# infergo-ml/gogp

Hardware: AMD Instinct MI355X
Metric: GP.Observe+Gradient evals/sec (fp64) at N=16384 D=8 (higher is better)
Workload: dtype f64

## Files before the change

gogp_amd/_lib.py:

```python
from __future__ import annotations

import ctypes
import os
import subprocess

from .kernel import CDesc

_HERE = os.path.dirname(os.path.abspath(__file__))
LIB_PATH = os.path.join(_HERE, "libgogp_hip.so")
HOOKS_PATH = os.path.join(_HERE, "libgogp_testhooks.so")

GOGP_OK, GOGP_EARG, GOGP_ENOTPD, GOGP_EHIP, GOGP_ESTATE, GOGP_ENOMEM, GOGP_ECOND = 0, 1, 2, 3, 4, 5, 6
GOGP_MAX_CANDIDATES = 16
GOGP_BATCH_MAX_N = 128
GOGP_COV_MAX_M = 4096

_dp = ctypes.POINTER(ctypes.c_double)
_i64 = ctypes.c_int64
_h = ctypes.c_void_p
_descp = ctypes.POINTER(CDesc)
GOGP_UNIQUE_ID_BYTES = 128


class CXfer(ctypes.Structure):
    _fields_ = [("peer", ctypes.c_int32), ("is_send", ctypes.c_int32), ("buf", ctypes.c_void_p),
                ("bytes", ctypes.c_int64)]


EXCHANGE_FN = ctypes.CFUNCTYPE(ctypes.c_int, ctypes.c_void_p, ctypes.POINTER(CXfer), ctypes.c_int32)
ALLREDUCE_FN = ctypes.CFUNCTYPE(ctypes.c_int, ctypes.c_void_p, ctypes.POINTER(ctypes.c_double),
                                ctypes.c_int64)
class CGemmOpts(ctypes.Structure):
    _fields_ = [(n, ctypes.c_int32) for n in ("ktri", "krag0", "new_row0", "kbeg0", "small_below", "prio", "rule",
                                              "tpb_shift", "rblk0", "cblk0", "pr", "Pr", "pc", "Pc", "beta0", "k")]
    _fields_ += [("bstride", ctypes.c_int64)]
    DEFAULTS = dict(ktri=0, krag0=-1, new_row0=-1, kbeg0=0, small_below=384, prio=0, rule=0, tpb_shift=0, rblk0=0,
                    cblk0=0, pr=0, Pr=1, pc=0, Pc=1, beta0=-1, k=1, bstride=0)


class CKParams(ctypes.Structure):
    _T, _D, _E = 4, 64, 32
    _fields_ = [("ndim", ctypes.c_int32), ("nterms", ctypes.c_int32), ("kind", ctypes.c_int32 * _T),
                ("ard", ctypes.c_int32 * _T), ("c", ctypes.c_double * _T), ("w", ctypes.c_double * _T),
                ("inv_len", (ctypes.c_double * _D) * _T), ("noise_var", ctypes.c_double), ("dnoise", ctypes.c_double),
                ("nevents", ctypes.c_int32), ("ev_axis", ctypes.c_int32), ("ev_from", ctypes.c_double * _E),
                ("ev_to", ctypes.c_double * _E), ("ev_disc", ctypes.c_double * _E)]


GOGP_TEST_NACC = 16 + 64


class CGemmPlan(ctypes.Structure):
    _fields_ = [("tile", ctypes.c_int32), ("waves", ctypes.c_int32), ("grid_x", ctypes.c_int64),
                ("grid_z", ctypes.c_int64), ("flops", ctypes.c_double), ("tag", ctypes.c_int64)]


SYMBOLS = [
    ("gogp_desc_check", ctypes.c_int, [_descp]),
    ("gogp_desc_ntheta_noise", ctypes.c_int, [_descp]),
    ("gogp_create", ctypes.c_int, [_descp, ctypes.c_int, ctypes.POINTER(_h)]),
    ("gogp_destroy", None, [_h]),
    ("gogp_last_error", ctypes.c_char_p, [_h]),
    ("gogp_notpd_index", _i64, [_h]),
    ("gogp_graph_info", ctypes.c_int, [_h, ctypes.POINTER(ctypes.c_int64), ctypes.POINTER(ctypes.c_int)]),
    ("gogp_events_check", ctypes.c_int, [_dp, ctypes.c_int, ctypes.c_int, ctypes.c_int]),
    ("gogp_set_events", ctypes.c_int, [_h, _dp, ctypes.c_int, ctypes.c_int]),
    ("gogp_set_data", ctypes.c_int, [_h, _dp, _dp, _i64]),
    ("gogp_set_data_device", ctypes.c_int, [_h, ctypes.c_void_p, ctypes.c_void_p, _i64]),
    ("gogp_absorb", ctypes.c_int, [_h, _dp, _dp]),
    ("gogp_observe", ctypes.c_int, [_h, _dp, _i64, _dp]),
    ("gogp_observe_full", ctypes.c_int, [_h, _dp, _i64, _dp]),
    ("gogp_lml", ctypes.c_int, [_h, _dp]),
    ("gogp_gradient", ctypes.c_int, [_h, _dp, _i64]),
    ("gogp_loo", ctypes.c_int, [_h, _dp, _dp, _dp, _dp]),
    ("gogp_loo_gradient", ctypes.c_int, [_h, _dp, _i64]),
    ("gogp_observe_gradient_batch", ctypes.c_int,
     [ctypes.POINTER(_h), ctypes.c_int, _dp, _i64, _dp, _dp, ctypes.POINTER(ctypes.c_int)]),
    ("gogp_observe_gradient_candidates", ctypes.c_int,
     [_h, ctypes.c_int, _dp, _i64, _dp, _dp, ctypes.POINTER(ctypes.c_int)]),
    ("gogp_batch_set_data", ctypes.c_int,
     [_h, _dp, _dp, _i64, ctypes.c_int32, ctypes.POINTER(_i64), ctypes.POINTER(_i64)]),
    ("gogp_batch_observe_gradient", ctypes.c_int,
     [_h, ctypes.c_int32, ctypes.POINTER(ctypes.c_int32), _dp, _i64, _dp, _dp, ctypes.POINTER(ctypes.c_int)]),
    ("gogp_batch_produce", ctypes.c_int,
     [_h, ctypes.c_int32, ctypes.POINTER(ctypes.c_int32), _dp, _i64, ctypes.POINTER(_i64), _dp, _dp, _dp, _dp,
      ctypes.POINTER(ctypes.c_int)]),
    ("gogp_batch_observe_full_gradient", ctypes.c_int,
     [_h, ctypes.c_int32, _dp, ctypes.POINTER(_i64), _dp, _dp, ctypes.POINTER(ctypes.c_int)]),
    ("gogp_batch_produce_full", ctypes.c_int,
     [_h, ctypes.c_int32, _dp, ctypes.POINTER(_i64), ctypes.POINTER(_i64), _dp, _dp, _dp, _dp,
      ctypes.POINTER(ctypes.c_int)]),
    ("gogp_produce", ctypes.c_int, [_h, _dp, _i64, _dp, _dp]),
    ("gogp_produce_gradient", ctypes.c_int, [_h, _dp, _i64, _dp, _dp, _dp, _dp]),
    ("gogp_produce_covariance", ctypes.c_int, [_h, _dp, _i64, _dp, _dp]),
    ("gogp_produce_samples", ctypes.c_int, [_h, _dp, _i64, _dp, _i64, ctypes.c_double, _dp, _dp]),
    ("gogp_n", _i64, [_h]),
    ("gogp_get_alpha", ctypes.c_int, [_h, _dp]),
    ("gogp_get_factor", ctypes.c_int, [_h, _dp]),
    ("gogp_get_factor_rows", ctypes.c_int, [_h, ctypes.POINTER(_i64), _i64, _dp]),
    ("gogp_get_factor_diag", ctypes.c_int, [_h, _dp]),
    ("gogp_set_factor", ctypes.c_int, [_h, _dp, _dp, _dp, _dp]),
    ("gogp_append", ctypes.c_int, [_h, _dp, _dp, ctypes.c_int64]),
    ("gogp_remove", ctypes.c_int, [_h, ctypes.POINTER(_i64), ctypes.c_int64]),
    ("gogp_dist_grid", ctypes.c_int, [ctypes.c_int, ctypes.POINTER(ctypes.c_int), ctypes.POINTER(ctypes.c_int)]),
    ("gogp_dist_unique_id", ctypes.c_int, [ctypes.c_void_p]),
    ("gogp_dist_init_rccl", ctypes.c_int,
     [_h, ctypes.c_int, ctypes.c_int, ctypes.c_int, ctypes.c_int, ctypes.c_char_p]),
    ("gogp_dist_init_callbacks", ctypes.c_int,
     [_h, ctypes.c_int, ctypes.c_int, ctypes.c_int, ctypes.c_int, ctypes.c_void_p, ctypes.c_void_p,
      ctypes.c_void_p]),
    ("gogp_dist_local_bytes", _i64, [_h]),
    ("gogp_dist_comm_ranks", ctypes.c_int, [_h, ctypes.POINTER(ctypes.c_int)]),
    ("gogp_dist_selftest", ctypes.c_int, [_h, ctypes.c_int, _i64]),
    ("gogp_profile_enable", ctypes.c_int, [_h, ctypes.c_int]),
    ("gogp_profile_read", ctypes.c_int, [_h, _dp, ctypes.POINTER(_i64), _dp, _dp]),
    ("gogp_profile_read_launches", ctypes.c_int,
     [_h, _i64, _dp, _dp, _dp, ctypes.POINTER(_i64), ctypes.POINTER(_i64)]),
    ("gogp_profile_read_aux", ctypes.c_int, [_h, ctypes.c_int, _dp, ctypes.POINTER(_i64)]),
    ("gogp_set_option", ctypes.c_int, [_h, ctypes.c_char_p, _i64]),
    ("gogp_version", ctypes.c_char_p, []),
]

HOOK_SYMBOLS = [
    ("gogp_mfma_f64_peak", ctypes.c_int, [ctypes.c_int, ctypes.c_int, _dp, _dp, _dp]),
    ("gogp_mfma_f32_peak", ctypes.c_int, [ctypes.c_int, ctypes.c_int, _dp, _dp, _dp]),
    ("gogp_bench_gemm", ctypes.c_int,
     [ctypes.c_int, ctypes.c_int, ctypes.c_int, ctypes.c_int, _i64, ctypes.c_int, _dp, _dp]),
    ("gogp_test_diag256", ctypes.c_int,
     [ctypes.c_int, _dp, _dp, _dp, ctypes.POINTER(ctypes.c_uint64), _dp]),
    ("gogp_test_dgemm_nt", ctypes.c_int,
     [ctypes.c_int, _i64, _i64, _i64, ctypes.c_double, _dp, _dp, ctypes.c_double, _dp]),
    ("gogp_test_valu_cost", ctypes.c_int, [ctypes.c_int, _dp]),
    ("gogp_test_panel128", ctypes.c_int,
     [ctypes.c_int, _dp, _dp, _i64, ctypes.c_int, ctypes.POINTER(ctypes.c_uint64), _dp]),
    ("gogp_test_panel128_slabs", ctypes.c_int, [ctypes.c_int, _dp, _dp, _i64, ctypes.c_int, ctypes.c_int, _dp]),
    ("gogp_test_gemm_nt", ctypes.c_int,
     [ctypes.c_int, ctypes.c_int, ctypes.c_int, ctypes.c_int, ctypes.c_int, _i64, ctypes.c_double, ctypes.c_double]
# ... 90 lines not shown
```

gogp_amd/csrc/api.hip:

```cpp
#include <math.h>
#include <stdio.h>
#include <stdlib.h>
#include <string.h>

#include <algorithm>
#include <initializer_list>
#include <mutex>
#include <new>
#include <thread>
#include <type_traits>
#include <utility>

#include "handle.h"

using namespace gogp;

static thread_local std::string g_create_error;

extern "C" int gogp_desc_ntheta_noise(const gogp_desc *d) {
  return (d && (d->noise_kind == GOGP_NOISE_UNIFORM || d->noise_kind == GOGP_NOISE_CONSTANT_PARAM)) ? 1 : 0;
}

extern "C" int gogp_desc_check(const gogp_desc *d) {
  if (!d) return GOGP_EARG;
// ... 537 lines not shown
  int P0, nsub, prevP0, next_nsub;
  int64_t C0() const { return (int64_t)P0 * PANEL; }
  int64_t CE() const { return C0() + (int64_t)nsub * PANEL; }
};
static std::vector<SuperPanel> superpanels(const gogp_handle *h) {
  const int npanel = (int)(h->npad / PANEL);
  std::vector<SuperPanel> v;
  for (int P0 = 0; P0 < npanel; P0 += v.back().nsub) {
    const int nsub = superpanel_width(h, npanel, P0);
    if (!v.empty()) v.back().next_nsub = nsub;
    v.push_back({P0, nsub, v.empty() ? -1 : v.back().P0, 0});
  }
  return v;
}
struct InnerGroup {
  int grp;
  int64_t k0, ce;
};
static inline InnerGroup inner_group(int q, int64_t c2, int64_t CE) {
  const int done = q + 1, grp = done & -done;
  return {grp, c2 - (int64_t)grp * PANEL, std::min(c2 + (int64_t)grp * PANEL, CE)};
}

constexpr int TMT_BLOCKS = 8;
static inline int tinv_panels(const gogp_handle *h) { return h->produce_panels; }
static inline int64_t tinv_signature(const gogp_handle *h) {
  return (int64_t)h->produce_panels + (h->npad << 8) + ((int64_t)h->prec << 56);
}
static int ensure_tinv(gogp_handle *h) {
  const int64_t tld = (int64_t)tinv_panels(h) * PANEL;
  const size_t need = (size_t)std::max(h->npad, h->cap_npad) * (size_t)tld;
  if (!h->TX || h->cap_tinv < need) {
    (void)hipFree(h->TX);
    (void)hipFree(h->Tmt);
    h->TX = h->Tmt = nullptr;
    h->cap_tinv = 0;
    HIPCHK(h, hipMalloc(&h->TX, need * h->esz()));
    HIPCHK(h, hipMalloc(&h->Tmt, (size_t)TMT_BLOCKS * PANEL * PANEL * h->esz()));
    h->cap_tinv = need;
  }
  h->tinv_ld = tld;
  return GOGP_OK;
}

template <class T>
static void assemble_tinv(gogp_handle *h, hipStream_t sp, int P0, int nsub) {
  const int64_t ld = h->npad, tld = h->tinv_ld, C0 = (int64_t)P0 * PANEL;
  T *X = reinterpret_cast<T *>(h->TX) + C0 * tld;
  T *MT = reinterpret_cast<T *>(h->Tmt);
  const T *L = reinterpret_cast<const T *>(h->bufL);
  const T *Dinv = reinterpret_cast<const T *>(h->Dinv) + (size_t)P0 * PANEL * PANEL;
  launch_tinv_init(sp, Dinv, X, (T *)nullptr, nsub, tld);
  for (int d = 1; d < nsub; ++d) {
    const int cnt = nsub - d;
    for (int b0 = 0; b0 < cnt; b0 += 6) {
      const int nb = std::min(6, cnt - b0);
      const T *A1[6], *B1[6], *A2[6], *B2[6];
      T *C1[6], *C2[6];
      int64_t lda1[6], ldb1[6], ldc1[6], lda2[6], ldb2[6], ldc2[6];
      int K1[6], K2[6];
      for (int b = 0; b < nb; ++b) {
        const int i = d + b0 + b, j = i - d;
        A1[b] = L + (C0 + (int64_t)i * PANEL) * ld + C0 + (int64_t)j * PANEL;
        lda1[b] = ld;
        B1[b] = X + (int64_t)j * PANEL * tld + (int64_t)j * PANEL;
        ldb1[b] = tld;
        C1[b] = MT + (size_t)(b0 + b) * PANEL * PANEL;
        ldc1[b] = PANEL;
        K1[b] = d * PANEL;
        A2[b] = Dinv + (size_t)i * PANEL * PANEL;
        lda2[b] = PANEL;
        B2[b] = C1[b];
        ldb2[b] = PANEL;
        C2[b] = X + (int64_t)i * PANEL * tld + (int64_t)j * PANEL;
        ldc2[b] = tld;
        K2[b] = PANEL;
      }
      launch_blockmm(sp, nb, A1, lda1, B1, ldb1, C1, ldc1, K1, 1.0);
      launch_blockmm(sp, nb, A2, lda2, B2, ldb2, C2, ldc2, K2, -1.0);
    }
  }
}

template <class T>
struct InvBufs {
  T *A, *Y;
  const T *L, *Dinv;
};
template <class T>
static void trtri_superstep(gogp_handle *h, const InvBufs<T> &B, const SuperPanel &P, hipStream_t st, hipStream_t s2) {
  const int64_t npad = h->npad, ld = npad;
  T *R = B.A, *Y = B.Y;
  const T *L = B.L;
  GemmProfile *pf = &h->prof;
  const int P0 = P.P0;
  const int64_t C0 = P.C0(), CE = P.CE();
  for (int q = 0; q < P.nsub; ++q) {
    const int p = P0 + q;
    const int64_t c0 = (int64_t)p * PANEL, c2 = c0 + PANEL;
    const T *Dp = B.Dinv + (size_t)p * PANEL * PANEL;
    launch_ydiag(st, Dp, Y + c0 * ld + c0, ld);
    if (c2 < CE)
      launch_zero_block(st, Y + c2 * ld + c0, ld, CE - c2, PANEL);
    if (c0 > 0) {
      GemmGrid gtri = chain_grid(h);
      gtri.ktri = h->ktri;
      launch_gemm_nt(st, GEMM_RECT, (int)(c0 / TILE), 2, PANEL, 1.0, R + c0, ld, Dp, PANEL, 0.0,
                      Y + c0, ld, pf, &gtri);
    }
    if (c2 < CE) {
      const InnerGroup g = inner_group(q, c2, CE);
      GemmGrid gch = chain_grid(h);
      if (h->krag) gch.krag0 = (int)(g.k0 / TILE);
      launch_gemm_nt(st, GEMM_RECT, (int)(c2 / TILE), (int)((g.ce - c2) / TILE), (int64_t)g.grp * PANEL,
                      -1.0, Y + g.k0, ld, L + c2 * ld + g.k0, ld, 1.0, R + c2, ld, pf, &gch);
    }
  }
  order(h, EV_BASE + 4 * P0 + 2, st, s2);
  const int nt = (int)((npad - CE) / TILE);
  if (nt > 0) {
    const int64_t Kw = CE - C0;
    const int mr = (int)(CE / TILE);
    const int ntn = nt < 2 * P.next_nsub ? nt : 2 * P.next_nsub;
    if (P0 > 0 && st != s2)
      (void)gogp::rec_stream_wait(st, ev(h, EV_BASE + 4 * P.prevP0 + 3));
    GemmGrid gch = chain_grid(h), gbulk;
    if (h->krag) gch.krag0 = gbulk.krag0 = (int)(C0 / TILE);
    launch_gemm_nt(st, GEMM_RECT, mr, ntn, Kw, -1.0, Y + C0, ld, L + CE * ld + C0, ld, 1.0,
                    R + CE, ld, pf, &gch);
    if (nt > ntn) {
      const int64_t C3 = CE + (int64_t)ntn * TILE;
      launch_gemm_nt(s2, GEMM_RECT, mr, nt - ntn, Kw, -1.0, Y + C0, ld, L + C3 * ld + C0, ld, 1.0,
                      R + C3, ld, pf, &gbulk);
    }
    (void)gogp::rec_event_record(ev(h, EV_BASE + 4 * P0 + 3), s2);
  }
}

static inline bool mixed_gradient(const gogp_handle *h) {
  return h->grad_prec == 32 && h->prec == 64 && !h->batch_mode && !h->dist;
}
static int ensure_g32(gogp_handle *h) {
  const int64_t cap = std::max(h->npad, h->cap_npad);
  if (h->g32A && h->g32_cap >= cap) return GOGP_OK;
  (void)hipFree(h->g32A);
  (void)hipFree(h->g32L);
  (void)hipFree(h->g32Y);
  (void)hipFree(h->g32D);
  h->g32A = h->g32L = h->g32Y = h->g32D = nullptr;
  h->g32_cap = 0;
  const size_t nn = (size_t)cap * (size_t)cap * sizeof(float);
  HIPCHK(h, hipMalloc(&h->g32A, nn));
  HIPCHK(h, hipMalloc(&h->g32L, nn));
  HIPCHK(h, hipMalloc(&h->g32Y, nn));
  HIPCHK(h, hipMalloc(&h->g32D, (size_t)(cap / PANEL) * PANEL * PANEL * sizeof(float)));
  h->g32_cap = cap;
  return GOGP_OK;
}
static void mixed_superstep(gogp_handle *h, const SuperPanel &P, hipStream_t st, hipStream_t s2) {
  const int64_t npad = h->npad, ld = npad, C0 = P.C0(), W = P.CE() - C0;
  launch_convert_block(st, h->bufL + C0 * ld + C0, ld, h->g32L + C0 * ld + C0, ld, (int)(npad - C0), (int)W);
  launch_convert_block(st, h->Dinv + (size_t)P.P0 * PANEL * PANEL, PANEL, h->g32D + (size_t)P.P0 * PANEL * PANEL, PANEL,
                       (int)W, PANEL);
  const InvBufs<float> B{h->g32A, h->g32Y, h->g32L, h->g32D};
  trtri_superstep<float>(h, B, P, st, s2);
}

template <class T>
static void kinv_accumulate(gogp_handle *h, const T *Y, T *A, int64_t C0, int64_t CE) {
  (void)gogp::rec_stream_wait(h->sk, ev(h, EV_BASE + 4 * (size_t)(C0 / PANEL) + 2));
  GemmGrid gk;
  gk.new_row0 = (int)(C0 / TILE);
  if (h->krag) gk.krag0 = (int)(C0 / TILE);
  launch_gemm_nt(h->sk, GEMM_LOWER, (int)(CE / TILE), (int)(CE / TILE), CE - C0, 1.0, Y + C0, h->npad, Y + C0, h->npad,
                 1.0, A, h->npad, &h->prof, &gk);
}

template <class T>
static void zero_inverse_rhs(gogp_handle *h, bool mixed, hipStream_t s) {
  if (mixed)
    launch_zero_upper_blocks(s, h->g32A, h->npad, h->npad);
  else
    launch_zero_upper_blocks(s, reinterpret_cast<T *>(h->bufA), h->npad, h->npad);
}
template <class T>
static void inverse_superstep(gogp_handle *h, bool mixed, const SuperPanel &P, hipStream_t st, hipStream_t s2,
                              bool fuse_kinv) {
  if (mixed) {
    mixed_superstep(h, P, st, s2);
    if (fuse_kinv) kinv_accumulate<float>(h, h->g32Y, h->g32A, P.C0(), P.CE());
  } else {
    const InvBufs<T> B{reinterpret_cast<T *>(h->bufA), reinterpret_cast<T *>(h->bufY), reinterpret_cast<const T *>(h->bufL),
                       reinterpret_cast<const T *>(h->Dinv)};
    trtri_superstep<T>(h, B, P, st, s2);
    if (fuse_kinv) kinv_accumulate<T>(h, B.Y, B.A, P.C0(), P.CE());
  }
}

static inline int chain_split_of(const gogp_handle *h, bool eager) {
  if (h->dist || h->prec != 64) return 0;
  if (h->chain_split >= 0) return h->chain_split;
  return (h->npad <= 8192 || !eager) ? 2 : 0;
}
static void fused_panel(gogp_handle *h, hipStream_t sp, double *A, double *L, int64_t ld, int64_t c0, int64_t npad,
                        GemmProfile *pf) {
  const int64_t c1 = c0 + TILE, c2 = c0 + PANEL;
  const int mt1 = (int)((npad - c1) / TILE);
  const GemmGrid gch = chain_grid(h);
  launch_panel128_slabs(sp, A + c0 * ld + c0, ld, L + c0 * ld + c0, ld, 0, npad - c1, c0, h->n, h->info, h->chain_slabs);
  launch_gemm_nt(sp, GEMM_RECT, mt1, 1, TILE, -1.0, L + c1 * ld + c0, ld, L + c1 * ld + c0, ld, 1.0, A + c1 * ld + c1, ld,
                 pf, &gch);
  launch_panel128_slabs(sp, A + c0 * ld + c0, ld, L + c0 * ld + c0, ld, 1, npad - c2, c0, h->n, h->info, h->chain_slabs);
}

static void begin_evaluation(gogp_handle *h, std::initializer_list<hipStream_t> streams) {
  auto wait = [&](int e) {
    for (hipStream_t q : streams) (void)gogp::rec_stream_wait(q, ev(h, e));
  };
  if (h->trtri_pending) wait(EV_TRTRI);
  if (h->kinv_pending) wait(EV_KINV);
  if (h->kinv_c1 > 0 && !h->have_kinv) wait(EV_KINV);
  h->trtri_pending = h->kinv_pending = false;
  h->factored = h->have_alpha = h->have_kinv = h->grad_valid = false;
  h->alpha_pending = h->trtri_done = h->ydone_valid = h->d64_active = false;
  h->notpd = -1;
  h->kinv_c1 = 0;
  if (!h->batch_mode) h->tinv_valid = false;
}
static hipError_t enqueue_result_scalars(gogp_handle *h, hipStream_t s) {
  const hipError_t e = cand_d2h(h, h->hscal, h->scalars, 7 * sizeof(double), s);
  return e != hipSuccess ? e : cand_d2h(h, h->hscal + HS_INFO, h->info, sizeof(long long), s);
}

template <class T>
static void substitute_fwd(gogp_handle *h, hipStream_t q, const T *L, const T *Dinv, double *w, double *dst) {
  const int npanel = (int)(h->npad / PANEL);
  for (int b = 0; b < npanel; ++b) launch_trsv_fwd_step(q, L, h->npad, Dinv, b, npanel, w, dst);
}
template <class T>
static hipError_t substitute_bwd(gogp_handle *h, hipStream_t q, const T *L, const T *Dinv, const double *src, double *w,
                                 double *dst) {
  const int npanel = (int)(h->npad / PANEL);
  const hipError_t e = hipMemcpyAsync(w, src, (size_t)h->npad * sizeof(double), hipMemcpyDeviceToDevice, q);
  for (int b = npanel - 1; b >= 0 && e == hipSuccess; --b) launch_trsv_bwd_step(q, L, h->npad, Dinv, b, npanel, w, dst);
  return e;
}

template <class T>
struct Sweep {
  static constexpr bool fp32 = sizeof(T) == 4;
  gogp_handle *h;
  bool eager;
  T *A = reinterpret_cast<T *>(h->bufA), *L = reinterpret_cast<T *>(h->bufL), *Dinv = reinterpret_cast<T *>(h->Dinv);
  int64_t npad = h->npad, ld = npad;
  int npanel = (int)(npad / PANEL);
  GemmProfile *pf = &h->prof;
  hipStream_t s = h->s, st = h->st, s2 = h->s2;
  hipStream_t sp = h->lookahead ? h->sp : h->s;
  hipStream_t sz = h->lookahead ? h->sl : sp;
  bool mixed = !fp32 && mixed_gradient(h);
  bool fuse_kinv = eager && (h->kinv_fused < 0 ? (npad <= 10240 || mixed) : h->kinv_fused != 0);
  int split = fp32 ? 0 : chain_split_of(h, eager);

  void d64_init(hipStream_t q, int first, int nblk) const {
    if constexpr (fp32)
      launch_widen_diag_blocks(q, A + (int64_t)first * PANEL * (ld + 1), ld, h->D64 + (size_t)first * PANEL * PANEL, nblk);
  }
  void d64_update(hipStream_t q, int64_t k0, int64_t K, int first, int nblk) const {
    if constexpr (fp32) {
      if (h->d64_active)
        launch_diag_syrk_f64(q, L + (int64_t)first * PANEL * ld + k0, ld, K, h->D64 + (size_t)first * PANEL * PANEL, nblk);
    }
  }

  int build_gram() const {
    if (sp != s) order(h, EV_ENTRY, s, sp);
    HIPCHK(h, cand_memset(h, h->info, sizeof(long long), sp));
    const int w0 = superpanel_width(h, npanel, 0);
    {
      AuxTimer tm(h, GOGP_PROF_GRAM, s);
      launch_gram_lower_split(sp, s, h->devP, h->D, h->dX, h->n, npad, A, ld, (int64_t)w0 * PANEL, h->ev());
    }
    h->d64_active = fp32 && h->diag_fp64 != 0;
    if (h->d64_active) {
      const int rc = ensure_d64(h);
      if (rc != GOGP_OK) return rc;
      d64_init(sp, 0, w0);
      if (npanel > w0) d64_init(s, w0, npanel - w0);
    }
    (void)gogp::rec_event_record(ev(h, EV_GRAM), s);
    if (eager) {
      (void)gogp::rec_stream_wait(s2, ev(h, EV_GRAM));
      (void)gogp::rec_stream_wait(st, ev(h, EV_GRAM));
      zero_inverse_rhs<T>(h, mixed, s2);
      order(h, EV_INIT, s2, st);
    }
    return GOGP_OK;
  }

  void chain_superpanel(const SuperPanel &P) const {
    const int64_t CE = P.CE();
    for (int q = 0; q < P.nsub; ++q) {
      const int p = P.P0 + q;
      const int64_t c0 = (int64_t)p * PANEL, c2 = c0 + PANEL;
      if constexpr (!fp32) {
        if (split) fused_panel(h, sp, A, L, ld, c0, npad, pf);
      }
      if (!split) {
        T *Dp = Dinv + (size_t)p * PANEL * PANEL;
        diag_block(h, sp, A + c0 * ld + c0, ld, L + c0 * ld + c0, ld, Dp, c0);
        const int mt2 = (int)((npad - c2) / TILE);
        if (mt2 > 0) {
          GemmGrid gtri = chain_grid(h);
          gtri.ktri = h->ktri;
          launch_gemm_nt(sp, GEMM_RECT, mt2, 2, PANEL, 1.0, A + c2 * ld + c0, ld, Dp, PANEL, 0.0,
                          L + c2 * ld + c0, ld, pf, &gtri);
        }
      }
      if (c2 < CE) {
        d64_update(sp, c0, PANEL, p + 1, (int)((CE - c2) / PANEL));
        const InnerGroup g = inner_group(q, c2, CE);
        const GemmGrid gch = chain_grid(h);
        launch_gemm_nt(sp, GEMM_TRAP, (int)((npad - c2) / TILE), (int)((g.ce - c2) / TILE),
                        (int64_t)g.grp * PANEL, -1.0, L + c2 * ld + g.k0, ld, L + c2 * ld + g.k0, ld, 1.0,
                        A + c2 * ld + c2, ld, pf, &gch);
      }
    }
  }

  void panels_final(const SuperPanel &P) const {
    order(h, EV_BASE + 4 * P.P0, sp, s);
    if (sz != sp) (void)gogp::rec_stream_wait(sz, ev(h, EV_BASE + 4 * P.P0));
    if constexpr (!fp32) {
      if (split) {
        launch_dinv256_blocks(sz, L + (int64_t)P.P0 * PANEL * (ld + 1), ld, Dinv + (size_t)P.P0 * PANEL * PANEL, P.nsub);
        if (eager) {
          (void)gogp::rec_event_record(ev(h, EV_BASE + 5 * (size_t)npanel + 32 + (size_t)P.P0), sz);
          (void)gogp::rec_stream_wait(st, ev(h, EV_BASE + 5 * (size_t)npanel + 32 + (size_t)P.P0));
        }
      }
    }
    for (int q = 0; q < P.nsub; ++q) launch_trsv_fwd_step(sz, L, ld, Dinv, P.P0 + q, npanel, h->w, h->z);
  }

  void trailing_update(const SuperPanel &P) const {
    const int64_t C0 = P.C0(), CE = P.CE();
    const int mtE = (int)((npad - CE) / TILE);
    if (mtE <= 0) return;
    const int64_t Kw = CE - C0;
    const int ntn = mtE < 2 * P.next_nsub ? mtE : 2 * P.next_nsub;
    (void)gogp::rec_stream_wait(sp, ev(h, P.P0 > 0 ? EV_BASE + 4 * P.prevP0 + 1 : EV_GRAM));
    const GemmGrid gch = chain_grid(h);
    launch_gemm_nt(sp, GEMM_TRAP, mtE, ntn, Kw, -1.0, L + CE * ld + C0, ld, L + CE * ld + C0, ld,
                    1.0, A + CE * ld + CE, ld, pf, &gch);
    d64_update(sp, C0, Kw, (int)(CE / PANEL), ntn / 2);
    if (mtE > ntn) {
      const int64_t C3 = CE + (int64_t)ntn * TILE;
      launch_gemm_nt(s, GEMM_LOWER, mtE - ntn, mtE - ntn, Kw, -1.0, L + C3 * ld + C0, ld,
                      L + C3 * ld + C0, ld, 1.0, A + C3 * ld + C3, ld, pf);
      d64_update(s, C0, Kw, (int)(C3 / PANEL), (mtE - ntn) / 2);
    }
    (void)gogp::rec_event_record(ev(h, EV_BASE + 4 * P.P0 + 1), s);
  }

  void inverse_behind(const SuperPanel &P) const {
    const int64_t CE = P.CE();
    (void)gogp::rec_stream_wait(st, ev(h, EV_BASE + 4 * P.P0));
    inverse_superstep<T>(h, mixed, P, st, s2, fuse_kinv);
    if (!fp32 && !fuse_kinv && !mixed && !h->batch_mode && h->kinv_split > 0 && h->kinv_c1 == 0 && CE < npad &&
        CE * 100 >= npad * (int64_t)h->kinv_split) {
      (void)gogp::rec_stream_wait(h->sk, ev(h, EV_BASE + 4 * P.P0 + 2));
      const T *Y0 = reinterpret_cast<const T *>(h->bufY);
      launch_gemm_nt(h->sk, GEMM_LAUUM, (int)(CE / TILE), (int)(CE / TILE), CE, 1.0, Y0, ld, Y0, ld, 0.0, A, ld, pf);
      (void)gogp::rec_event_record(ev(h, EV_KINV), h->sk);
      h->kinv_c1 = CE;
    }
  }

  int finish_alpha() const {
    if (fp32) {
      if (sz != sp) (void)gogp::rec_stream_wait(sp, ev(h, EV_FWD));
      HIPCHK(h, substitute_bwd(h, sp, L, Dinv, h->z, h->w, h->alpha));
      for (int it = 0; it < h->refine_steps; ++it) {
        launch_residual(sp, h->devP, h->D, h->dX, h->n, npad, h->alpha, h->dy, h->rpart, REFINE_SLABS, h->rw,
                        h->radial1, h->ev());
        substitute_fwd(h, sp, L, Dinv, h->rw, h->rz);
        HIPCHK(h, substitute_bwd(h, sp, L, Dinv, h->rz, h->rw, h->rd));
        launch_axpy(sp, h->alpha, h->rd, npad);
      }
      launch_dot(sp, h->dy, h->alpha, h->n, h->scalars + 6);
      order(h, EV_ALPHA, sp, s);
    }
    HIPCHK(h, enqueue_result_scalars(h, s));
    if (fp32) {
      if (eager) (void)gogp::rec_event_record(ev(h, EV_TRTRI), st);
    } else if (eager && !mixed) {
      (void)gogp::rec_stream_wait(st, ev(h, EV_FWD));
      launch_alpha_from_y(st, reinterpret_cast<const T *>(h->bufY), ld, h->z, npad, h->alpha);
      (void)gogp::rec_event_record(ev(h, EV_ALPHA), st);
      (void)gogp::rec_event_record(ev(h, EV_TRTRI), st);
    } else {
      if (sz != sp) (void)gogp::rec_stream_wait(sp, ev(h, EV_FWD));
      HIPCHK(h, substitute_bwd(h, sp, L, Dinv, h->z, h->w, h->alpha));
      (void)gogp::rec_event_record(ev(h, EV_ALPHA), sp);
    }
    return GOGP_OK;
  }
};

template <class T>
static int factorize_t(gogp_handle *h, bool eager) {
  const Sweep<T> c{h, eager && h->lookahead != 0};
  begin_evaluation(h, {c.s, c.sp});
  int rc = gogp_upload_params(h);
  if (rc == GOGP_OK && (c.mixed || c.eager)) rc = c.mixed ? ensure_g32(h) : ensure_y(h);
  if (rc == GOGP_OK) rc = c.build_gram();
  if (rc != GOGP_OK) return rc;
  if (c.fp32) HIPCHK(h, hipMemsetAsync(h->scalars + 5, 0, sizeof(double), c.sp));
  HIPCHK(h, cand_copy_in(h, h->w, h->dy, (size_t)c.npad * sizeof(double), c.sp));
  if (c.sz != c.sp) order(h, EV_W, c.sp, c.sz);
  for (const SuperPanel &P : superpanels(h)) {
    c.chain_superpanel(P);
    c.panels_final(P);
    c.trailing_update(P);
    if (c.eager) c.inverse_behind(P);
  }
  if (c.fuse_kinv) {
    (void)gogp::rec_event_record(ev(h, EV_KINV), h->sk);
    h->kinv_pending = true;
  }
  if (c.eager) {
    (void)gogp::rec_event_record(ev(h, EV_TRTRI), c.st);
    (void)gogp::rec_event_record(ev(h, EV_YDONE), c.st);
    h->ydone_valid = h->trtri_done = h->trtri_pending = true;
  }
  order(h, EV_FWD, c.sz, c.s);
  launch_lml_scalars(c.s, c.L, c.ld, h->z, nullptr, nullptr, h->n, h->scalars);
  rc = c.finish_alpha();
  if (rc != GOGP_OK) return rc;
  const int rcf = finish_factorize(h, c.fp32, c.fp32, false);
  if (rcf == GOGP_ENOTPD)
    for (hipStream_t q : {c.sp, c.st, c.s2, h->sl, h->sk}) (void)hipStreamSynchronize(q);
  return rcf;
}

static inline bool tiny_ok(const gogp_handle *h) {
  return h->tiny && !h->dist && h->prec == 64 && h->npad == PANEL && h->n <= TILE && !mixed_gradient(h);
}
static int tiny_factorize(gogp_handle *h, bool eager) {
  hipStream_t s = h->s;
  begin_evaluation(h, {s});
  int rc = gogp_upload_params(h);
  if (rc != GOGP_OK) return rc;
  if (h->lookahead && !h->batch_mode) {
    order(h, EV_ENTRY, h->sp, s);
    order(h, EV_W, h->sl, s);
  }
  HIPCHK(h, cand_memset(h, h->info, sizeof(long long), s));
  launch_tiny_eval(s, h->devP, h->dX, h->dy, h->n, h->bufA, h->bufL, h->Dinv, h->z, h->alpha, h->info, eager, h->ev());
  launch_lml_scalars(s, h->bufL, h->npad, h->z, nullptr, nullptr, h->n, h->scalars);
  (void)gogp::rec_event_record(ev(h, EV_ALPHA), s);
  HIPCHK(h, enqueue_result_scalars(h, s));
  return finish_factorize(h, false, false, eager);
}

static int factorize(gogp_handle *h, bool eager) {
  if (tiny_ok(h)) return tiny_factorize(h, eager && h->lookahead);
  return h->prec == 32 ? factorize_t<float>(h, eager) : factorize_t<double>(h, eager);
}

static int ensure_alpha(gogp_handle *h) {
  if (!h->factored || !h->have_alpha) return fail(h, GOGP_ESTATE, "no factorisation");
  if (h->alpha_pending) {
    HIPCHK(h, gogp::rec_stream_wait(h->s, ev(h, EV_ALPHA)));
    h->alpha_pending = false;
  }
  return GOGP_OK;
}

static const char *theta_refusal(const gogp_handle *h, const double *ts, const double *tn) {
  for (int i = 0; i < h->ns; ++i)
    if (!(ts[i] > 0.0) || !std::isfinite(ts[i])) return "similarity parameters must be positive and finite";
  for (int i = 0; i < h->nn; ++i)
    if (!std::isfinite(tn[i])) return "noise parameter must be finite";
  return nullptr;
}

static int set_theta_natural(gogp_handle *h, const double *ts, const double *tn) {
  if (const char *why = theta_refusal(h, ts, tn)) return fail(h, GOGP_EARG, why);
  for (int i = 0; i < h->ns; ++i) h->theta_s[i] = ts[i];
  for (int i = 0; i < h->nn; ++i) h->theta_n[i] = tn[i];
  h->have_theta = true;
  return GOGP_OK;
}

extern "C" int gogp_absorb(gogp_handle *h, const double *theta_simil,
                           const double *theta_noise) {
  if (!h || !theta_simil || (h->nn > 0 && !theta_noise)) return fail(h, GOGP_EARG, "absorb: NULL");
  if (!h->have_data) return fail(h, GOGP_ESTATE, "absorb: no data (gogp_set_data)");
  HIPCHK(h, hipSetDevice(h->device));
  int rc = set_theta_natural(h, theta_simil, theta_noise);
// ... 7 lines not shown
    return GOGP_OK;
  }
  rc = h->dist ? gogp_dist_factorize(h, false) : factorize(h, false);
  if (rc != GOGP_OK && rc != GOGP_ECOND) return rc;
  const int rcond = rc;
  rc = ensure_alpha(h);
  if (rc != GOGP_OK) return rc;
  HIPCHK(h, hipStreamSynchronize(h->s));
  return rcond;
}

static int observe_theta(gogp_handle *h, const double *x, double *lml) {
  std::vector<double> th(h->P > 0 ? h->P : 1);
  for (int i = 0; i < h->P; ++i) th[i] = exp(x[i]);
  int rc = set_theta_natural(h, th.data(), th.data() + h->ns);
  if (rc != GOGP_OK) return rc;
  h->grad_valid = false;
  if (h->n == 0) {
    h->lml = 0.0;
    h->factored = false;
    h->observed = true;
    if (lml) *lml = 0.0;
    return GOGP_OK;
  }
  rc = h->dist ? gogp_dist_factorize(h, true)
               : factorize(h, h->eager != 0);
  if (rc != GOGP_OK && rc != GOGP_ECOND) return rc;
  h->observed = true;
  if (lml) *lml = h->lml;
  return rc;
}

extern "C" int gogp_observe(gogp_handle *h, const double *x, int64_t len, double *lml) {
  if (!h || !x) return fail(h, GOGP_EARG, "observe: NULL");
  if (len != h->P) return fail(h, GOGP_EARG, "len(x)");
  if (!h->have_data) return fail(h, GOGP_ESTATE, "observe: no data (gogp_set_data)");
  HIPCHK(h, hipSetDevice(h->device));
  h->with_obs = false;
  return observe_theta(h, x, lml);
}

extern "C" int gogp_observe_full(gogp_handle *h, const double *x, int64_t len, double *lml) {
  if (!h || !x) return fail(h, GOGP_EARG, "observe: NULL");
  if (len < h->P) return fail(h, GOGP_EARG, "len(x)");
  const int64_t rest = len - h->P;
  if (rest == 0) return gogp_observe(h, x, len, lml);
  const int64_t n = rest / (h->D + 1);
  if (n * (h->D + 1) != rest) return fail(h, GOGP_EARG, "len(x)");
  int rc = gogp_set_data(h, x + h->P, x + h->P + n * h->D, n);
  if (rc != GOGP_OK) return rc;
  h->with_obs = true;
  return observe_theta(h, x, lml);
}

extern "C" int gogp_lml(gogp_handle *h, double *lml) {
  if (!h || !lml) return GOGP_EARG;
  if (h->n == 0) {
    *lml = 0.0;
    return GOGP_OK;
  }
  if (!h->factored) return fail(h, GOGP_ESTATE, "LML: nothing absorbed");
  *lml = h->lml;
  return GOGP_OK;
}

template <class T>
static int compute_kinv_t(gogp_handle *h) {
  if (h->have_kinv) return GOGP_OK;
  const int64_t npad = h->npad, ld = npad;
  hipStream_t s = h->s;
  GemmProfile *pf = &h->prof;
  if (h->kinv_pending) {
    (void)gogp::rec_stream_wait(s, ev(h, EV_KINV));
    if (h->trtri_pending) (void)gogp::rec_stream_wait(s, ev(h, EV_TRTRI));
    h->kinv_pending = h->trtri_pending = false;
    h->have_kinv = true;
    return GOGP_OK;
  }
  const bool mixed = std::is_same<T, double>::value && mixed_gradient(h);
  if (!h->trtri_done) {
    hipStream_t sp = h->lookahead ? h->sp : h->s;
    const int rcy = mixed ? ensure_g32(h) : ensure_y(h);
    if (rcy != GOGP_OK) return rcy;
    zero_inverse_rhs<T>(h, mixed, s);
    order(h, EV_INIT, s, sp);
    for (const SuperPanel &P : superpanels(h)) inverse_superstep<T>(h, mixed, P, sp, s, false);
    order(h, EV_TRTRI, sp, s);
    h->trtri_done = true;
  } else if (h->trtri_pending) {
    (void)gogp::rec_stream_wait(s, ev(h, h->ydone_valid ? EV_YDONE : EV_TRTRI));
  }
  if (mixed) {
    launch_gemm_nt(s, GEMM_LAUUM, h->nblk, h->nblk, npad, 1.0, h->g32Y, ld, h->g32Y, ld, 0.0, h->g32A, ld, pf);
  } else {
    GemmGrid gk;
    if (h->kinv_c1 > 0) {
      (void)gogp::rec_stream_wait(s, ev(h, EV_KINV));
      gk.kbeg0 = (int)h->kinv_c1;
    }
    launch_gemm_nt(s, GEMM_LAUUM, h->nblk, h->nblk, npad, 1.0, reinterpret_cast<const T *>(h->bufY), ld,
                   reinterpret_cast<const T *>(h->bufY), ld, 0.0, reinterpret_cast<T *>(h->bufA), ld, pf, &gk);
  }
  if (h->trtri_pending && h->ydone_valid) (void)gogp::rec_stream_wait(s, ev(h, EV_TRTRI));
  h->trtri_pending = false;
  h->have_kinv = true;
  return GOGP_OK;
}
static int compute_kinv(gogp_handle *h) {
  return h->prec == 32 ? compute_kinv_t<float>(h) : compute_kinv_t<double>(h);
}

static int64_t grad_len(const gogp_handle *h) {
  return h->with_obs ? h->P + h->n * (h->D + 1) : h->P;
}

static void assemble_gradient(const gogp_handle *h, const double *a, double dnoise, double *out) {
  const gogp_desc &d = h->desc;
  for (int t = 0; t < d.nterms; ++t) {
    const gogp_term &T = d.terms[t];
    if (T.scale_idx >= 0) out[T.scale_idx] += 0.5 * a[3 * t + 0];
    if (T.ard) {
      for (int j = 0; j < d.ndim; ++j) out[T.len_idx + j] += 0.5 * a[ACC_ARD0 + j];
    } else {
      out[T.len_idx] += 0.5 * a[3 * t + 1];
    }
    if (T.kind == GOGP_K_PERIODIC) out[T.period_idx] += 0.5 * a[3 * t + 2];
  }
  if (h->nn > 0) out[h->ns] = 0.5 * a[ACC_TRACE] * dnoise;
}

static void fp32_gradient_identities(const gogp_handle *h, double *a, double trace_w, double yta, double noise_var) {
  const gogp_desc &d = h->desc;
  a[ACC_TRACE] = trace_w;
  if (d.nterms == 1 && d.terms[0].scale_idx >= 0) a[0] = (yta - (double)h->n) - noise_var * trace_w;
}

static int enqueue_grad_sums(gogp_handle *h, bool trace) {
  hipStream_t s = h->s;
  auto reduce = [&](auto *kinv) {
    AuxTimer tm(h, GOGP_PROF_GRAD, s);
    launch_grad_reduce(s, h->devP, h->D, h->ard_dims, h->dX, h->alpha, kinv, h->npad, h->n, h->npad, h->gpart, h->gout,
                       h->radial1, h->ard_mfma_min, h->ev());
  };
  if (h->prec == 32)
    reduce(reinterpret_cast<const float *>(h->bufA));
  else if (mixed_gradient(h))
    reduce((const float *)h->g32A);
  else
    reduce((const double *)h->bufA);
  HIPCHK(h, cand_d2h(h, h->hscal + HS_GRAD, h->gout, NACC * sizeof(double), s));
  h->hscal[HS_TRACE] = NAN;
  if (trace) {
    launch_trace_from_y(s, h->prec == 32 ? reinterpret_cast<const float *>(h->bufY) : (const float *)h->g32Y, h->npad, h->n,
                        h->npad, h->alpha, h->prec == 32 ? h->rw : h->w, h->scalars + 7);
    HIPCHK(h, hipMemcpyAsync(h->hscal + HS_TRACE, h->scalars + 7, sizeof(double), hipMemcpyDeviceToHost, s));
  }
  return GOGP_OK;
}

extern "C" int gogp_gradient(gogp_handle *h, double *grad, int64_t len) {
  if (!h || !grad) return fail(h, GOGP_EARG, "gradient: NULL");
  if (!h->observed) return fail(h, GOGP_ESTATE, "Gradient before Observe");
  if (len != grad_len(h)) return fail(h, GOGP_EARG, "gradient: wrong length");
  for (int64_t i = 0; i < len; ++i) grad[i] = 0.0;
  if (h->n == 0) return GOGP_OK;
  HIPCHK(h, hipSetDevice(h->device));
  if (h->dist && h->with_obs)
    return fail(h, GOGP_EARG, "sharded evaluation: the full Observe form is not supported");
  if (h->prec == 32 && h->with_obs)
// ... 1598 lines not shown
    h->trtri_done = h->trtri_pending = h->kinv_pending = false;
    return GOGP_OK;
  }
  if (strcmp(name, "trace_fp64") == 0) {
    h->trace_fp64 = value != 0;
    return GOGP_OK;
  }
  if (strcmp(name, "krag") == 0) {
    h->krag = value != 0;
    return GOGP_OK;
  }
  if (strcmp(name, "lookahead") == 0) {
    h->lookahead = value != 0;
    return GOGP_OK;
  }
  if (strcmp(name, "eager") == 0) {
    h->eager = value != 0;
    return GOGP_OK;
  }
  if (strcmp(name, "precision") == 0) {
    if (value != 32 && value != 64) return fail(h, GOGP_EARG, "precision must be 32 or 64");
    if (h->dist && (int)value != h->prec)
      return fail(h, GOGP_EARG, "precision: set it before gogp_dist_init_* (the shard's buffers are typed)");
    if ((int)value != h->prec) {
      HIPCHK(h, hipSetDevice(h->device));
      for (hipStream_t q : work_streams(h)) HIPCHK(h, hipStreamSynchronize(q));
      free_n_buffers(h);
      free_m_buffers(h);
      free_cand_buffers(h);
      h->prec = (int)value;
      h->have_data = h->factored = h->have_alpha = h->have_kinv = h->observed = h->grad_valid = false;
      h->trtri_done = h->trtri_pending = h->alpha_pending = h->kinv_pending = false;
    }
    return GOGP_OK;
  }
  if (strcmp(name, "kinv_split") == 0) {
    if (value < 0 || value > 95) return fail(h, GOGP_EARG, "kinv_split must be 0..95");
    h->kinv_split = (int)value;
    return GOGP_OK;
  }
  if (strcmp(name, "kinv_fused") == 0) {
    h->kinv_fused = value < 0 ? -1 : (value != 0);
    return GOGP_OK;
  }
  if (strcmp(name, "superpanel_head") == 0) {
    if (value < -1 || value > 8) return fail(h, GOGP_EARG, "superpanel_head must be -1..8");
    h->superpanel_head = (int)value;
    return GOGP_OK;
  }
  if (strcmp(name, "head_remaining") == 0) {
    if (value < 0) return fail(h, GOGP_EARG, "head_remaining must be >= 0");
    h->head_remaining = (int)value;
    return GOGP_OK;
  }
  if (strcmp(name, "ard_mfma_min_dims") == 0) {
    if (value < 1 || value > 65) return fail(h, GOGP_EARG, "ard_mfma_min_dims must be 1..65");
    h->ard_mfma_min = (int)value;
    return GOGP_OK;
  }
  if (strcmp(name, "chain_prio") == 0) {
    if (value < -1 || value > 2) return fail(h, GOGP_EARG, "chain_prio must be -1..2");
    h->chain_prio = (int)value;
    return GOGP_OK;
  }
  if (strcmp(name, "tiny") == 0) {
    if (value < 0 || value > 1) return fail(h, GOGP_EARG, "tiny must be 0 or 1");
    h->tiny = (int)value;
    return GOGP_OK;
  }
  if (strcmp(name, "chain_slabs") == 0) {
    if (value < 0 || value > 8) return fail(h, GOGP_EARG, "chain_slabs must be 0..8");
    h->chain_slabs = (int)value;
    return GOGP_OK;
  }
  if (strcmp(name, "chain_split") == 0) {
    if (value < -1 || value > 2 || value == 1) return fail(h, GOGP_EARG, "chain_split must be -1, 0 or 2");
    h->chain_split = (int)value;
    return GOGP_OK;
  }
  if (strcmp(name, "ktri") == 0) {
    h->ktri = value != 0;
    return GOGP_OK;
  }
  if (strcmp(name, "graph") == 0) {
    if (value < 0 || value > 3) return fail(h, GOGP_EARG, "graph must be 0..3");
    h->use_graph = (int)value;
    h->graph_failed = false;
    drop_cand_graph(h);
    return GOGP_OK;
  }
  if (strcmp(name, "diag_fp64") == 0) {
    if (value < 0 || value > 1) return fail(h, GOGP_EARG, "diag_fp64 must be 0 or 1");
    h->diag_fp64 = (int)value;
    return GOGP_OK;
  }
  if (strcmp(name, "refine_steps") == 0) {
    if (value < 0 || value > 8) return fail(h, GOGP_EARG, "refine_steps must be 0..8");
    h->refine_steps = (int)value;
    return GOGP_OK;
  }
  if (strcmp(name, "cond_limit_log10") == 0) {
    if (value < 1 || value > 300) return fail(h, GOGP_EARG, "cond_limit_log10 must be 1..300");
    h->cond_limit = pow(10.0, (double)value);
    return GOGP_OK;
  }
  if (strcmp(name, "superpanel") == 0) {
    if (value < 1 || value > 8) return fail(h, GOGP_EARG, "superpanel must be 1..8");
    h->superpanel = (int)value;
    return GOGP_OK;
  }
  return fail(h, GOGP_EARG, "unknown option");
}
```

gogp_amd/csrc/common.h:

```cpp
#pragma once
#include <hip/hip_runtime.h>
#include <stdint.h>

#include <string>
#include <vector>

#include "../../include/gogp_hip.h"
#include "graphrec.h"

namespace gogp {

constexpr int TILE = 128;
constexpr int PANEL = 256;
constexpr int GEMM_BK = 16;

struct DevParams {
  int ndim, nterms, ns, nn;
  int kind[GOGP_MAX_TERMS];
  int ard[GOGP_MAX_TERMS];
  double c[GOGP_MAX_TERMS];
  double w[GOGP_MAX_TERMS];
  double inv_len[GOGP_MAX_TERMS][GOGP_MAX_NDIM];
  double noise_var;
  double dnoise;
  int nevents, ev_axis;
  double ev_from[GOGP_MAX_EVENTS], ev_to[GOGP_MAX_EVENTS], ev_disc[GOGP_MAX_EVENTS];
};

constexpr int ACC_TRACE = 3 * GOGP_MAX_TERMS;
constexpr int ACC_ARD0 = 16;
constexpr int NACC = ACC_ARD0 + GOGP_MAX_NDIM;

struct Batch {
  int k = 1;
  long stride = 0;
};
inline thread_local Batch tl_batch;
template <class P>
__device__ __forceinline__ P *cand(P *p, long bstride) {
  return (P *)((const char *)p + (long)blockIdx.z * bstride);
}

struct GemmProfile {
  bool on = false;
  std::vector<hipEvent_t> pool;
  size_t used = 0;
  double flops = 0;
  int64_t launches = 0;
  std::vector<double> lflops;
  std::vector<int64_t> ltag;
};

struct GemmGrid {
  int rule = 0, tpb_shift = 0, rblk0 = 0, cblk0 = 0, pr = 0, Pr = 1, pc = 0, Pc = 1, beta0 = -1;
  int new_row0 = -1;
  int ktri = 0;
  int prio = 0;
  int krag0 = -1;
  int small_below = 384;
  int kbeg0 = 0;
};

struct BlockMap {
  int nb_shift = 9, pr = 0, Pr = 1, pc = 0, Pc = 1;
  __host__ __device__ long grow(long lrow) const {
    const long nbm = (1L << nb_shift) - 1;
    return ((((lrow >> nb_shift) * Pr + pr)) << nb_shift) + (lrow & nbm);
  }
  __host__ __device__ long gcol(long lcol) const {
    const long nbm = (1L << nb_shift) - 1;
    return ((((lcol >> nb_shift) * Pc + pc)) << nb_shift) + (lcol & nbm);
  }
};

#ifdef GOGP_WGSTAMP
struct StampRec {
  long long base, nwg, tag, stream;
};
constexpr int STAMP_SLOTS = 8;
extern unsigned long long *g_stamp_buf;
extern long long g_stamp_cap, g_stamp_used, g_stamp_nrec;
extern StampRec g_stamp_rec[1 << 16];
unsigned long long *stamp_reserve(long long nwg, long long tag, hipStream_t s);
#endif

enum GemmMode { GEMM_RECT = 0, GEMM_LOWER = 1, GEMM_LAUUM = 2,
                GEMM_TRAP = 3 };

void launch_dgemm_nt(hipStream_t s, GemmMode mode, int mt, int nt, int64_t K,
                     double alpha, const double *A, int64_t lda, const double *B,
                     int64_t ldb, double beta, double *C, int64_t ldc,
                     GemmProfile *prof, const GemmGrid *grid = nullptr);

void launch_gemm_nt(hipStream_t s, GemmMode mode, int mt, int nt, int64_t K, double alpha, const double *A,
                    int64_t lda, const double *B, int64_t ldb, double beta, double *C, int64_t ldc,
                    GemmProfile *prof, const GemmGrid *grid = nullptr);
void launch_gemm_nt(hipStream_t s, GemmMode mode, int mt, int nt, int64_t K, double alpha, const float *A,
                    int64_t lda, const float *B, int64_t ldb, double beta, float *C, int64_t ldc,
                    GemmProfile *prof, const GemmGrid *grid = nullptr);
void launch_gram_lower_split(hipStream_t s_first, hipStream_t s_rest, const DevParams *p, int ndim,
                             const double *X, int64_t n, int64_t npad, float *K, int64_t ld,
                             int64_t wcols, bool ev = false);
void launch_cross(hipStream_t s, const DevParams *p, int ndim, const double *X, int64_t n,
                  int64_t npad, const double *Z, int64_t m, int64_t mpad, float *KsT, int64_t ld, bool ev = false);
void launch_trsv_fwd_step(hipStream_t s, const float *L, int64_t ld, const float *Dinv, int b, int nblk,
                          double *y, double *z);
void launch_trsv_bwd_step(hipStream_t s, const float *L, int64_t ld, const float *Dinv, int b, int nblk,
                          double *zwork, double *alpha);
void launch_lml_scalars(hipStream_t s, const float *L, int64_t ld, const double *z, const double *y,
                        const double *alpha, int64_t n, double *scalars);
void launch_alpha_from_y(hipStream_t s, const float *Y, int64_t ld, const double *z, int64_t npad,
                         double *alpha);
void launch_rownorm_dot(hipStream_t s, const float *V, int64_t ld, const double *vec, int64_t ncols,
                        int64_t m, double *dot, double *sq);
void launch_zero_upper_blocks(hipStream_t s, float *R, int64_t ld, int64_t npad);
void launch_zero_block(hipStream_t s, float *B, int64_t ld, int64_t rows, int64_t cols);
void launch_ydiag(hipStream_t s, const float *Dinv, float *Ydiag, int64_t ld);
void launch_extract_lower(hipStream_t s, const float *L, int64_t ld, int64_t n, double *out);
void launch_pack_lower(hipStream_t s, const double *in, int64_t n, int64_t npad, float *L, int64_t ld);
void launch_convert_block(hipStream_t s, const float *src, int64_t lds_, double *dst, int64_t ldd, int rows,
                          int cols);
void launch_convert_block(hipStream_t s, const double *src, int64_t lds_, float *dst, int64_t ldd, int rows,
                          int cols);
void launch_grad_reduce(hipStream_t s, const DevParams *p, int ndim, int ard_dims, const double *X,
                        const double *alpha, const float *Kinv, int64_t ld, int64_t n, int64_t npad,
                        double *partials, double *out, bool radial1 = false, int mfma_min_dims = 1, bool ev = false,
                        int max_blocks = 0);

void launch_gram_lower(hipStream_t s, const DevParams *p, int ndim, const double *X,
                       int64_t n, int64_t npad, double *K, int64_t ld, bool ev = false);
void launch_gram_local(hipStream_t s, const DevParams *p, int ndim, const double *X, int64_t n,
                       int64_t mrows, int64_t ncols, BlockMap map, double *K, int64_t ld, bool ev = false);
void launch_gram_local(hipStream_t s, const DevParams *p, int ndim, const double *X, int64_t n,
                       int64_t mrows, int64_t ncols, BlockMap map, float *K, int64_t ld, bool ev = false);
void launch_gram_lower_split(hipStream_t s_first, hipStream_t s_rest, const DevParams *p, int ndim,
                             const double *X, int64_t n, int64_t npad, double *K, int64_t ld,
                             int64_t wcols, bool ev = false);
void launch_cross(hipStream_t s, const DevParams *p, int ndim, const double *X, int64_t n,
                  int64_t npad, const double *Z, int64_t m, int64_t mpad, double *KsT,
                  int64_t ld, bool ev = false);
void launch_residual(hipStream_t s, const DevParams *p, int ndim, const double *X, int64_t n, int64_t npad,
                     const double *v, const double *y, double *part, int nslab, double *r, bool radial1 = false,
                     bool ev = false);
void launch_kmatvec_share(hipStream_t s, const DevParams *p, int ndim, const double *X, int64_t n, int64_t npad,
                          const double *v, int part_idx, int nparts, double *part, int nslab, double *out,
                          bool radial1 = false, bool ev = false);
void launch_prior(hipStream_t s, const DevParams *p, const double *Z, int64_t m,
                  double *prior);

void launch_trsv_fwd_step(hipStream_t s, const double *L, int64_t ld, const double *Dinv,
                          int b, int nblk, double *y, double *z);
void launch_trsv_bwd_step(hipStream_t s, const double *L, int64_t ld, const double *Dinv,
                          int b, int nblk, double *zwork, double *alpha);

void launch_lml_scalars(hipStream_t s, const double *L, int64_t ld, const double *z,
                        const double *y, const double *alpha, int64_t n, double *scalars);
void launch_diag256(hipStream_t s, const double *A, int64_t ld, double *Lout, int64_t ldl,
                    double *Dinv, int64_t row0, int64_t nvalid, long long *info);
void launch_diag256_ld512(hipStream_t s, const double *A, int64_t ld, double *Lout, int64_t ldl,
                          double *Dinv, int64_t row0, int64_t nvalid, long long *info);
void launch_diag256_inv_only(hipStream_t s, const double *L, int64_t ld, double *Dinv);
void launch_diag_syrk_f64(hipStream_t s, const float *Lrows, int64_t ld, int64_t K, double *D64, int nblocks);
void launch_widen_diag_blocks(hipStream_t s, const float *A, int64_t ld, double *D64, int nblocks);
void launch_diag_syrk_f64_tiles(hipStream_t s, const float *Lrows, int64_t ld, int64_t K, double *D64, int nblocks,
                                int64_t row_stride, int bs);
void launch_panel128(hipStream_t s, const double *A, int64_t ld, double *Lout, int64_t ldl, int half, int64_t rows_below,
                     int64_t row0, int64_t nvalid, long long *info);
void launch_panel128_slabs(hipStream_t s, const double *A, int64_t ld, double *Lout, int64_t ldl, int half,
                           int64_t rows_below, int64_t row0, int64_t nvalid, long long *info, int slabs);
void launch_tiny_eval(hipStream_t s, const DevParams *P, const double *X, const double *y, int64_t n, double *A, double *L,
                      double *Dinv, double *z, double *alpha, long long *info, bool want_kinv, bool ev = false);
struct BatchItem {
  DevParams P;
  long off, n;
  long zoff, m;
  long roff;
};
constexpr int BATCH_ROW = NACC + 16;
void launch_batch_eval(hipStream_t s, const BatchItem *items, int k, const double *X, const double *y, const double *Z,
                       double *rows, double *mu, double *sigma, int ard_dims, bool produce, bool ev);
void launch_batch_eval_full(hipStream_t s, const BatchItem *items, int k, const double *x, const double *Z, double *rows,
                            double *mu, double *sigma, int ard_dims, bool produce, bool ev);
void launch_dinv256_blocks(hipStream_t s, const double *L, int64_t ld, double *Dinv, int nblk);
void launch_diag256_inv_only_ld512(hipStream_t s, const double *L, int64_t ld, double *Dinv);
void launch_convert_block(hipStream_t s, const double *src, int64_t lds_, double *dst, int64_t ldd, int rows,
                          int cols);
void launch_pack_lower(hipStream_t s, const double *in, int64_t n, int64_t npad, double *L,
                       int64_t ld);
void launch_sigma(hipStream_t s, const double *prior, const double *q, int64_t m,
                  double *sigma);
void launch_bwd_panel(hipStream_t s, int64_t rows16, const double *A, int64_t lda, const double *B, int64_t ldb,
                      double *C, int64_t ldc, int64_t ncols, int K, bool tri, bool sub);
int pgrad_slabs(int64_t npad, int64_t m, int *tiles_per_slab);
void launch_pgrad(hipStream_t s, const DevParams *p, int ndim, const double *X, int64_t n, int64_t npad,
                  const double *Z, int64_t m, const double *alpha, const double *Wt, int64_t ld, const double *sigma,
                  double *part, double *dmu, double *dsigma, bool ev);
int pcov_slabs(int64_t npad, int64_t m, int ncu, int *cols_per_slab);
void launch_pcov(hipStream_t s, const DevParams *p, const double *Z, int64_t m, const double *Vt, int64_t ld,
                 int64_t npad, int ncu, double *part, double diag_add, double *out, int64_t mo, int64_t ldo, bool ev);
void launch_pcov_add_mu(hipStream_t s, const double *G, int64_t ldg, const double *mu, int64_t ns, int64_t m, double *out);
int grad_reduce_blocks(int64_t npad);

void launch_grad_reduce(hipStream_t s, const DevParams *p, int ndim, int ard_dims,
                        const double *X, const double *alpha, const double *Kinv, int64_t ld, int64_t n,
                        int64_t npad, double *partials, double *out, bool radial1 = false, int mfma_min_dims = 1,
                        bool ev = false, int max_blocks = 0);
int grad_reduce_blocks_local(int64_t mrows, int64_t ncols);
void launch_grad_reduce_local(hipStream_t s, const DevParams *p, int ndim, int ard_dims,
                              const double *X, const double *alpha, const double *Kinv, int64_t ld,
                              int64_t n, int64_t mrows, int64_t ncols, BlockMap map, double *partials,
                              double *out, bool radial1 = false, int mfma_min_dims = 1, bool ev = false,
                              int max_blocks = 0);
void launch_grad_reduce_local(hipStream_t s, const DevParams *p, int ndim, int ard_dims,
                              const double *X, const double *alpha, const float *Kinv, int64_t ld,
                              int64_t n, int64_t mrows, int64_t ncols, BlockMap map, double *partials,
                              double *out, bool radial1 = false, int mfma_min_dims = 1, bool ev = false,
                              int max_blocks = 0);

void launch_grad_ard_mfma(hipStream_t s, const DevParams *p, int ndim, const double *X, const double *alpha,
                          const double *Kinv, int64_t ld, int64_t n, int nt, int ntc, int ntiles, int blocks,
                          BlockMap map, double *partials);
void launch_grad_ard_mfma(hipStream_t s, const DevParams *p, int ndim, const double *X, const double *alpha,
                          const float *Kinv, int64_t ld, int64_t n, int nt, int ntc, int ntiles, int blocks,
                          BlockMap map, double *partials);

void launch_xgrad(hipStream_t s, const DevParams *p, int ndim, const double *X,
                  const double *alpha, double *Kinv, int64_t ld, int64_t n, int64_t npad,
                  double *gx, bool ev = false);

void launch_rownorm_dot(hipStream_t s, const double *V, int64_t ld, const double *vec,
                        int64_t ncols, int64_t m, double *dot, double *sq);

void launch_zero_upper_blocks(hipStream_t s, double *R, int64_t ld, int64_t npad);
void launch_alpha_from_y(hipStream_t s, const double *Y, int64_t ld, const double *z,
                         int64_t npad, double *alpha);
void launch_zero_block(hipStream_t s, double *B, int64_t ld, int64_t rows, int64_t cols);
void launch_ydiag(hipStream_t s, const double *Dinv, double *Ydiag, int64_t ld);
void launch_tinv_init(hipStream_t s, const double *Dinv, double *X, double *XT, int nsub, int64_t tld);
void launch_tinv_init(hipStream_t s, const float *Dinv, float *X, float *XT, int nsub, int64_t tld);
void launch_blockmm(hipStream_t s, int nprod, const double *const *A, const int64_t *lda, const double *const *B,
                    const int64_t *ldb, double *const *C, const int64_t *ldc, const int *K, double alpha);
void launch_blockmm(hipStream_t s, int nprod, const float *const *A, const int64_t *lda, const float *const *B,
                    const int64_t *ldb, float *const *C, const int64_t *ldc, const int *K, double alpha);
void launch_trace_from_y(hipStream_t s, const float *Y, int64_t ld, int64_t n, int64_t npad, const double *alpha,
                         double *part, double *out);
size_t trsm_small_workspace_bytes(int64_t npad);
void launch_trsm_small(hipStream_t s, const double *L, int64_t ld, const double *Dinv, const double *KsT, int64_t ldk,
                       int64_t npad, int j0, int cnt, void *ws, double *dq, unsigned **tmo_dev);
void launch_trsm_small(hipStream_t s, const float *L, int64_t ld, const float *Dinv, const float *KsT, int64_t ldk,
                       int64_t npad, int j0, int cnt, void *ws, double *dq, unsigned **tmo_dev);
enum { TS_SOL_PAIRED = 0, TS_SOL_COMPACT = 1, TS_SOL_GRANULE = 2, TS_SOL_ROWS = 3 };
struct TsSolution {
  const void *p = nullptr;
  int kind = TS_SOL_PAIRED, width = 32;
};
TsSolution trsm_small_solution(int64_t npad, int j0, int cnt, void *ws, bool f32 = false);
constexpr int APPEND_PART = 64 * 64 + 64;
void launch_append_gram(hipStream_t s, TsSolution v0, TsSolution v1, int m0, int m, int64_t npc, int64_t n,
                        const double *z, double *part, double *Lnew, int64_t ld);
void launch_append_commit(hipStream_t s, const DevParams *p, const double *X2, const double *y2, int m, int64_t n,
                          const double *part, int nslab, double *Lnew, int64_t ld, double *z2out, long long *info,
                          bool ev);
void launch_append_identity_rows(hipStream_t s, double *L, int64_t ld, int64_t r0, int64_t r1, int64_t ncols);
void launch_append_restride(hipStream_t s, const double *src, int64_t ld0, int64_t npad0, double *dst, int64_t ld1,
                            int64_t npad1);
constexpr int REMOVE_W = 32, REMOVE_W_SMALL = 4;
void launch_remove_gather(hipStream_t s, const double *src, int64_t ld0, const int *map, int64_t n1, double *dst,
                          int64_t npad1);
void launch_remove_rows(hipStream_t s, const double *src, const int *map, int64_t n1, int width, double *dst);
void launch_remove_w(hipStream_t s, const double *src, int64_t ld0, const int *map, const int *rem, int mc, int mw, int64_t r0,
                     int64_t n1, int64_t npad1, double *W);
void launch_remove_snap(hipStream_t s, const double *L, int64_t ld, int b0, int nb, double *snap);
void launch_remove_block(hipStream_t s, double *L, int64_t ld, const double *snap, double *W, int mw, int64_t kb, int64_t n1);
void launch_loo_stats(hipStream_t s, const double *Kinv, int64_t ld, const double *alpha, const double *y, int64_t n,
                      int64_t npad, double *mu, double *sigma, double *logp, double *v, double *sc, double *part);
void launch_loo_scale_symv(hipStream_t s, const double *Kinv, int64_t ld, int64_t n, int64_t npad, const double *sc,
                           const double *v, double *B, int64_t ldb, double *upart, double *u);
void launch_loo_rank2(hipStream_t s, double *G, int64_t ld, int64_t n, int64_t npad, const double *u, const double *alpha);
void launch_fill(hipStream_t s, double *p, int64_t count, double v);
void launch_axpy(hipStream_t s, double *a, const double *b, int64_t count);
void launch_dot(hipStream_t s, const double *a, const double *b, int64_t n, double *out);
void launch_transpose_sq(hipStream_t s, const double *src, int64_t lds_, double *dst, int64_t ldd,
                         int n);
void launch_transpose_sq(hipStream_t s, const float *src, int64_t lds_, float *dst, int64_t ldd, int n);
void launch_pack_blocks(hipStream_t s, double *dst, const double *src, int nblk, int64_t blk,
                        int first, int stride);
int64_t chunk_tdot_scratch(int64_t max_rows, int nb);
void launch_chunk_tdot(hipStream_t s, const double *chunk, int64_t rows, int nb, const double *v,
                       double *part, double *out);
void launch_chunk_tdot(hipStream_t s, const float *chunk, int64_t rows, int nb, const double *v,
                       double *part, double *out);
void launch_chunk_alpha(hipStream_t s, const double *Ych, int mloc, int nloc, int nb, BlockMap map,
                        const double *z, double *out);
void launch_chunk_alpha(hipStream_t s, const float *Ych, int mloc, int nloc, int nb, BlockMap map,
                        const double *z, double *out);
void launch_chunk_sumsq(hipStream_t s, const double *Ych, int mloc, int nloc, int nb, BlockMap map, int64_t n, double *part,
                        double *out);
void launch_chunk_sumsq(hipStream_t s, const float *Ych, int mloc, int nloc, int nb, BlockMap map, int64_t n, double *part,
                        double *out);
void launch_logdet_block(hipStream_t s, const double *L, int64_t ld, int64_t row0, int64_t n, int nb,
                         double *acc);
void launch_sumsq_info(hipStream_t s, const double *z, int64_t n, const long long *info, double *out);
void launch_info_to_double(hipStream_t s, const long long *info, double *out);
void launch_extract_lower(hipStream_t s, const double *L, int64_t ld, int64_t n,
                          double *out);

}
```

gogp_amd/csrc/dgemm.hip:

```cpp
#include "gemm_tile.h"

namespace gogp {

typedef double f64x4 __attribute__((ext_vector_type(4)));
typedef double f64x2 __attribute__((ext_vector_type(2)));

#ifdef GOGP_WGSTAMP
unsigned long long *g_stamp_buf = nullptr;
long long g_stamp_cap = 0, g_stamp_used = 0, g_stamp_nrec = 0;
StampRec g_stamp_rec[1 << 16];
unsigned long long *stamp_reserve(long long nwg, long long tag, hipStream_t s) {
  if (!g_stamp_buf || g_stamp_used + nwg > g_stamp_cap || g_stamp_nrec >= (1 << 16)) return nullptr;
  unsigned long long *p = g_stamp_buf + STAMP_SLOTS * g_stamp_used;
  g_stamp_rec[g_stamp_nrec++] = {g_stamp_used, nwg, tag, (long long)(size_t)s};
  g_stamp_used += nwg;
  return p;
}
#define GOGP_STAMP_WG(k)                                                                                            \
  do {                                                                                                              \
    if (g.stamps && threadIdx.x == 0)                                                                               \
      g.stamps[((long)blockIdx.x + (long)gridDim.x * blockIdx.z) * STAMP_SLOTS + (k)] = __builtin_amdgcn_s_memrealtime(); \
  } while (0)
#else
#define GOGP_STAMP_WG(k) \
// ... 47 lines not shown
  __shared__ __attribute__((aligned(16))) double lds[2][2][BT * GEMM_BK];
  const int tid = threadIdx.x;
  const int lane = tid & 63;
  const int wid = __builtin_amdgcn_readfirstlane(tid >> 6);
  if (g.prio) raise_wave_priority();
  GOGP_STAMP_WG(0);
#ifdef GOGP_WGSTAMP
  if (g.stamps && threadIdx.x == 0) {
    unsigned long long *st = g.stamps + ((long)blockIdx.x + (long)gridDim.x * blockIdx.z) * STAMP_SLOTS;
    st[4] = __builtin_amdgcn_s_getreg((4 << 0) | (0 << 6) | (31 << 11));
    st[5] = __builtin_amdgcn_s_getreg((20 << 0) | (0 << 6) | (31 << 11));
  }
#endif

  int ti, tj, kbeg, nkt;
  double beta;
  if constexpr (MODE == GEMM_RECT) {
    if (!rect_tile_assignment<BT, GEMM_BK>(g, ti, tj, beta, kbeg, nkt)) return;
  } else {
    int t = blockIdx.x;
    if (MODE != GEMM_LAUUM) t = xcd_chunk(t);
    ti = (int)((sqrt(8.0 * (double)t + 1.0) - 1.0) * 0.5);
    while (ti * (ti + 1) / 2 > t) --ti;
    while ((ti + 1) * (ti + 2) / 2 <= t) ++ti;
    tj = t - ti * (ti + 1) / 2;
    beta = g.beta;
    if (MODE == GEMM_LOWER && ti >= g.new_row0) beta = 0.0;
    kbeg = 0, nkt = g.nkt;
    if (MODE != GEMM_LAUUM && ti > g.krag0) {
      kbeg = (ti - g.krag0) * BT;
      nkt -= kbeg / GEMM_BK;
    }
    if (MODE == GEMM_LAUUM) {
      kbeg = ti * BT;
      if (kbeg < g.kbeg0) {
        kbeg = g.kbeg0;
        beta = 1.0;
      }
      nkt = (g.kend - kbeg) / GEMM_BK;
      if (nkt <= 0) return;
    }
  }

  const double *Ag = cand(g.A, g.bstride) + (long)ti * BT * g.lda + kbeg;
  const double *Bg = cand(g.B, g.bstride) + (long)tj * BT * g.ldb + kbeg;

  const int srow = tid >> 3;
  const int schunk = tid & 7;
  const int gchunk = schunk ^ ((srow >> 1) & 7);
  const double *Ap = Ag + (long)srow * g.lda + gchunk * 2;
  const double *Bp = Bg + (long)srow * g.ldb + gchunk * 2;
  const long a_step = (long)SROWS * g.lda, b_step = (long)SROWS * g.ldb;

  const int wr = (NW == 8) ? wid >> 2 : wid >> 1;
  const int wc = (NW == 8) ? wid & 3 : wid & 1;
  const int frow = lane & 15;
  const int fk = lane >> 4;
  const int fchunk = fk >> 1;
  const int fhalf = fk & 1;
  const int abase = (wr * WT + frow) * GEMM_BK;
  const int bbase = (wc * WTN + frow) * GEMM_BK;
  unsigned afrag[4], bfrag[4];
  {
    const unsigned lds0 = lds_byte_address(&lds[0][0][0]);
#pragma unroll
    for (int kk = 0; kk < 4; ++kk) {
      const int xk = (((kk * 2 + fchunk) ^ ((frow >> 1) & 7)) << 1) + fhalf;
      afrag[kk] = lds0 + 8u * (unsigned)(abase + xk);
      bfrag[kk] = lds0 + 8u * (unsigned)(BT * GEMM_BK + bbase + xk);
    }
  }
  constexpr unsigned BUF_BYTES = 2u * BT * GEMM_BK * 8u;

  double *Cg = cand(g.C, g.bstride) + (long)(ti * BT + wr * WT) * g.ldc + tj * BT + wc * WTN;
  const int coff = (lane >> 4) * (int)g.ldc + (lane & 15);
  const double alpha = g.alpha;

#pragma unroll
  for (int q = 0; q < NQ; ++q) {
    load16_to_lds(Ap + q * a_step, &lds[0][0][(wid * 8 + SROWS * q) * GEMM_BK]);
    load16_to_lds(Bp + q * b_step, &lds[0][1][(wid * 8 + SROWS * q) * GEMM_BK]);
  }
  f64x4 acc[MT][NTW];
  if (beta != 0.0) {
    const double sc = beta / alpha;
#pragma unroll
    for (int m = 0; m < MT; ++m)
#pragma unroll
      for (int n = 0; n < NTW; ++n)
#pragma unroll
        for (int v = 0; v < 4; ++v)
          acc[m][n][v] = sc * (Cg + (long)(m * 16 + 4 * v) * g.ldc)[coff + n * 16];
  } else {
#pragma unroll
    for (int m = 0; m < MT; ++m)
#pragma unroll
      for (int n = 0; n < NTW; ++n) acc[m][n] = (f64x4){0.0, 0.0, 0.0, 0.0};
  }
  wait_vmcnt0();
  __syncthreads();
  GOGP_STAMP_WG(1);

  int cur = 0;
  for (int kt = 0; kt < nkt; ++kt) {
    const bool more = (kt + 1 < nkt);
    const unsigned curoff = (unsigned)cur * BUF_BYTES;
    double a[2][MT], b[2][NTW];
    read_frags<0, MT>(a[0], afrag[0] + curoff);
    read_frags<0, NTW>(b[0], bfrag[0] + curoff);
#pragma unroll
    for (int kk = 0; kk < 4; ++kk) {
      if (kk < 3) {
        read_frags<0, MT>(a[(kk + 1) & 1], afrag[kk + 1] + curoff);
        read_frags<0, NTW>(b[(kk + 1) & 1], bfrag[kk + 1] + curoff);
        lds_wait<MT + NTW>(a[kk & 1], b[kk & 1]);
      } else {
        lds_wait<0>(a[kk & 1], b[kk & 1]);
      }
#pragma unroll
      for (int m = 0; m < MT; ++m)
#pragma unroll
        for (int n = 0; n < NTW; ++n)
          acc[m][n] = __builtin_amdgcn_mfma_f64_16x16x4f64(a[kk & 1][m], b[kk & 1][n], acc[m][n], 0, 0, 0);
      sched_fence();
      if (kk == 0 && more) {
        const double *ap = Ap + (long)(kt + 1) * GEMM_BK;
        const double *bp = Bp + (long)(kt + 1) * GEMM_BK;
#pragma unroll
        for (int q = 0; q < NQ; ++q) {
          load16_to_lds(ap + q * a_step, &lds[cur ^ 1][0][(wid * 8 + SROWS * q) * GEMM_BK]);
          load16_to_lds(bp + q * b_step, &lds[cur ^ 1][1][(wid * 8 + SROWS * q) * GEMM_BK]);
        }
        sched_fence();
      }
    }
    if (more) wait_vmcnt0();
    __syncthreads();
    cur ^= 1;
  }

  GOGP_STAMP_WG(2);
#pragma unroll
  for (int m = 0; m < MT; ++m)
#pragma unroll
    for (int n = 0; n < NTW; ++n)
#pragma unroll
      for (int v = 0; v < 4; ++v)
        (Cg + (long)(m * 16 + 4 * v) * g.ldc)[coff + n * 16] = alpha * acc[m][n][v];
#ifdef GOGP_WGSTAMP
  if (g.stamps) {
    wait_vmcnt0();
    GOGP_STAMP_WG(3);
  }
#endif
}

template <>
struct TileKernel<double> {
  template <int MODE, int BT, int NW>
  static auto get() {
    return &dgemm_nt_kernel<MODE, BT, NW>;
  }
};

void launch_dgemm_nt(hipStream_t s, GemmMode mode, int mt, int nt, int64_t K, double alpha,
                     const double *A, int64_t lda, const double *B, int64_t ldb,
                     double beta, double *C, int64_t ldc, GemmProfile *prof, const GemmGrid *grid) {
  launch_tile_gemm<double>(s, mode, mt, nt, K, alpha, A, lda, B, ldb, beta, C, ldc, prof, grid);
}

}
```

gogp_amd/csrc/gemm_plan.h:

```cpp
#pragma once
#include <algorithm>

#include "common.h"

namespace gogp {

struct GemmPrecision {
  int kstep;
  bool band_513_768;
  bool cand_batch;
  bool lauum_kbeg0;
};
constexpr int SGEMM_BK = 32;
constexpr GemmPrecision GEMM_F64 = {GEMM_BK, true, true, true}, GEMM_F32 = {SGEMM_BK, false, false, false};

struct GemmPlan {
  int mt, nt, nkt, kend, trap, rule, tpb_shift, rblk0, cblk0, pr, Pr, pc, Pc, beta0, new_row0, ktri, prio, krag0;
  int kbeg0;
  GemmMode mode;
  int ntiles;
  double flops;
  int64_t tag;
  int tile, waves;
  unsigned gridx, gridz;
};

inline GemmPlan gemm_plan(GemmMode mode, int mt, int nt, int64_t K, const GemmGrid *grid, int ncand, GemmPrecision prec) {
  constexpr int NONE = 0x7fffffff;
  GemmPlan p{};
  if (!prec.cand_batch) ncand = 1;
  p.mt = mt;
  p.nt = nt;
  p.nkt = (int)(K / prec.kstep);
  p.kend = (int)K;
  p.trap = mode == GEMM_TRAP;
  p.rule = p.tpb_shift = p.rblk0 = p.cblk0 = p.pr = p.pc = p.beta0 = 0;
  p.Pr = p.Pc = 1;
  p.new_row0 = (mode == GEMM_LOWER && grid && grid->new_row0 >= 0) ? grid->new_row0 : NONE;
  p.ktri = (mode == GEMM_RECT && grid && grid->ktri) ? 1 : 0;
  p.prio = grid ? grid->prio : 0;
  p.krag0 = (mode != GEMM_LAUUM && mode != GEMM_TRAP && grid && grid->krag0 >= 0 && !p.ktri) ? grid->krag0 : NONE;
  p.kbeg0 = (mode == GEMM_LAUUM && grid && prec.lauum_kbeg0) ? grid->kbeg0 : 0;
  if (grid && grid->rule) {
    p.rule = grid->rule;
    p.tpb_shift = grid->tpb_shift;
    p.rblk0 = grid->rblk0;
    p.cblk0 = grid->cblk0;
    p.pr = grid->pr;
    p.Pr = grid->Pr;
    p.pc = grid->pc;
    p.Pc = grid->Pc;
    p.beta0 = grid->beta0;
  }
  int ntiles;
  double flops;
  if (mode == GEMM_TRAP) {
    mode = GEMM_RECT;
    ntiles = mt * nt;
    const int nb = nt / 2;
    flops = 2.0 * TILE * TILE * (double)K * ((double)mt * nt - 4.0 * nb * (nb - 1) / 2.0);
  } else if (mode == GEMM_RECT) {
    ntiles = mt * nt;
    flops = 2.0 * (double)mt * TILE * (double)nt * TILE * (double)K;
    if (p.ktri) {
      flops = 0;
      for (int j = 0; j < nt; ++j)
        flops += 2.0 * (double)mt * TILE * TILE * (double)std::min<int64_t>(K, (int64_t)(j + 1) * TILE);
    }
    if (p.krag0 != NONE) {
      flops = 0;
      for (int i = 0; i < mt; ++i)
        flops += 2.0 * (double)nt * TILE * TILE * (double)(K - (int64_t)std::max(0, i - p.krag0) * TILE);
    }
    if (p.rule) {
      const int tpb = 1 << p.tpb_shift;
      long kept = 0;
      for (int bi = 0; bi < mt / tpb; ++bi)
        for (int bj = 0; bj < nt / tpb; ++bj) {
          const int gI = (p.rblk0 + bi) * p.Pr + p.pr, gJ = (p.cblk0 + bj) * p.Pc + p.pc;
          kept += gI > gJ ? (long)tpb * tpb : (gI == gJ ? (long)tpb * (tpb + 1) / 2 : 0);
        }
      flops = 2.0 * (double)kept * TILE * TILE * (double)K;
    }
  } else {
    ntiles = mt * (mt + 1) / 2;
    if (mode == GEMM_LOWER && p.krag0 != NONE) {
      flops = 0;
      for (int i = 0; i < mt; ++i)
        flops += 2.0 * (double)(i + 1) * TILE * TILE * (double)(K - (int64_t)std::max(0, i - p.krag0) * TILE);
    } else if (mode == GEMM_LOWER) {
      flops = 2.0 * (double)ntiles * TILE * TILE * (double)K;
    } else {
      flops = 0;
      for (int i = 0; i < mt; ++i)
        flops += 2.0 * (double)(i + 1) * TILE * TILE * (double)(K - std::max<int64_t>((int64_t)i * TILE, p.kbeg0));
    }
  }
  p.mode = mode;
  p.ntiles = ntiles;
  p.flops = flops * ncand;
  p.tag = (int64_t)mode * 100000000LL + (int64_t)(K / 16) * 100000LL + (int64_t)std::min(ntiles, 99999);
  const long total_tiles = (long)ntiles * ncand;
  const bool small = (mode != GEMM_LAUUM) && (total_tiles < (grid ? grid->small_below : 384) ||
                                              (prec.band_513_768 && total_tiles > 512 && total_tiles <= 768));
  if (p.prio == 1 && !small) p.prio = 0;
  p.tile = small ? 64 : TILE;
  p.waves = (mode == GEMM_LAUUM || (!small && total_tiles >= 3072)) ? 8 : 4;
  p.gridx = p.rule ? 8 * ((mt + 7) / 8) * nt : ntiles;
  p.gridz = (unsigned)ncand;
  if (small) {
    p.mt = mt * 2;
    p.nt = nt * 2;
    p.tpb_shift += 1;
    if (p.new_row0 != NONE) p.new_row0 *= 2;
    if (p.krag0 != NONE) p.krag0 *= 2;
    p.gridx = (mode == GEMM_RECT) ? (p.rule ? 8 * ((p.mt + 7) / 8) * p.nt : p.mt * p.nt) : p.mt * (p.mt + 1) / 2;
  }
  return p;
}

}
```

gogp_amd/csrc/gemm_tile.h:

```cpp
#pragma once
#include <type_traits>

#include <hip/hip_ext.h>

#include "common.h"
#include "gemm_plan.h"

namespace gogp {

template <class T>
struct GemmArgsCommon {
  const T *A;
  const T *B;
  T *C;
  long lda, ldb, ldc;
  int mt, nt;
  int nkt;
  T alpha, beta;
  int kend;
  int trap;
  int rule, tpb_shift, rblk0, cblk0, pr, Pr, pc, Pc, beta0;
  int new_row0;
  int ktri;
  int prio;
  int krag0;
};
template <class T>
struct GemmArgs : GemmArgsCommon<T> {};
template <>
struct GemmArgs<double> : GemmArgsCommon<double> {
  int kbeg0;
  long bstride;
#ifdef GOGP_WGSTAMP
  unsigned long long *stamps;
#endif
};

template <class T>
__device__ __forceinline__ void load16_to_lds(const T *gsrc, T *lds_wave_base) {
#if defined(__HIP_DEVICE_COMPILE__)
  __builtin_amdgcn_global_load_lds(gsrc, lds_wave_base, 16, 0, 0);
#endif
}
__device__ __forceinline__ void raise_wave_priority() {
#if defined(__HIP_DEVICE_COMPILE__)
  __builtin_amdgcn_s_setprio(3);
#endif
}
__device__ __forceinline__ void wait_vmcnt0() {
#if defined(__HIP_DEVICE_COMPILE__)
  __builtin_amdgcn_s_waitcnt(0x0F70);
#endif
}

__device__ __forceinline__ int xcd_chunk(int t) {
  const int nwg = gridDim.x;
  const int q = nwg >> 3, r = nwg & 7;
  const int xcd = t & 7;
  return (xcd < r ? xcd * (q + 1) : r * (q + 1) + (xcd - r) * q) + (t >> 3);
}

template <int BT, int BK, class T>
__device__ __forceinline__ bool rect_tile_assignment(const GemmArgs<T> &g, int &ti_out, int &tj_out, T &beta_out,
                                                     int &kbeg_out, int &nkt_out) {
  int t = blockIdx.x;
  if (!g.rule) t = xcd_chunk(t);
  int ti, tj;
  if (g.rule) {
    const int x = t & 7, slot = t >> 3;
    const int rr = slot / g.nt;
    ti = x + 8 * rr;
    tj = slot - rr * g.nt;
    if (ti >= g.mt) return false;
  } else {
    ti = t / g.nt;
    tj = t - ti * g.nt;
    if (g.trap && (tj * BT) / PANEL > (ti * BT) / PANEL) return false;
  }
  T beta = g.beta;
  if (g.rule) {
    const int gI = (g.rblk0 + (ti >> g.tpb_shift)) * g.Pr + g.pr;
    const int gJ = (g.cblk0 + (tj >> g.tpb_shift)) * g.Pc + g.pc;
    const int msk = (1 << g.tpb_shift) - 1;
    if (gI < gJ || (gI == gJ && (ti & msk) < (tj & msk))) return false;
    if (g.rule == 2) beta = (gI == g.beta0) ? T(0) : T(1);
  }
  int kbeg = 0, nkt = g.nkt;
  if (g.ktri) nkt = min(nkt, (tj + 1) * BT / BK);
  if (ti > g.krag0) {
    kbeg = (ti - g.krag0) * BT;
    nkt -= kbeg / BK;
  }
  ti_out = ti, tj_out = tj, beta_out = beta, kbeg_out = kbeg, nkt_out = nkt;
  return true;
}

template <class T>
struct TileKernel;

template <class T>
void launch_tile_gemm(hipStream_t s, GemmMode mode, int mt, int nt, int64_t K, double alpha, const T *A, int64_t lda,
                      const T *B, int64_t ldb, double beta, T *C, int64_t ldc, GemmProfile *prof, const GemmGrid *grid) {
  if (mt <= 0 || nt <= 0 || K <= 0) return;
  constexpr bool F64 = std::is_same_v<T, double>;
  const GemmPlan p = gemm_plan(mode, mt, nt, K, grid, tl_batch.k, F64 ? GEMM_F64 : GEMM_F32);
  GemmArgs<T> g;
  g.A = A;
  g.B = B;
  g.C = C;
  g.lda = lda;
  g.ldb = ldb;
  g.ldc = ldc;
  g.alpha = (T)alpha;
  g.beta = (T)beta;
  g.mt = p.mt, g.nt = p.nt, g.nkt = p.nkt, g.kend = p.kend, g.trap = p.trap;
  g.rule = p.rule, g.tpb_shift = p.tpb_shift, g.rblk0 = p.rblk0, g.cblk0 = p.cblk0, g.beta0 = p.beta0;
  g.pr = p.pr, g.Pr = p.Pr, g.pc = p.pc, g.Pc = p.Pc;
  g.new_row0 = p.new_row0, g.ktri = p.ktri, g.prio = p.prio, g.krag0 = p.krag0;
  if constexpr (F64) {
    g.kbeg0 = p.kbeg0;
    g.bstride = tl_batch.stride;
#ifdef GOGP_WGSTAMP
    const int shape = p.tile == 64 ? 1 : (p.waves == 8 ? 3 : 2);
    g.stamps = stamp_reserve((long long)p.gridx * p.gridz, 10000000000LL * shape + p.tag, s);
#endif
  }
  hipEvent_t e0 = nullptr, e1 = nullptr;
  if (prof && prof->on) {
    if (prof->used + 2 > prof->pool.size()) {
      size_t old = prof->pool.size();
      prof->pool.resize(old + 1024);
      for (size_t i = old; i < prof->pool.size(); ++i) (void)hipEventCreate(&prof->pool[i]);
    }
    e0 = prof->pool[prof->used++];
    e1 = prof->pool[prof->used++];
    prof->flops += p.flops;
    prof->launches += 1;
    prof->lflops.push_back(p.flops);
    prof->ltag.push_back(p.tag);
  }
  using K_ = TileKernel<T>;
  void (*kernel)(GemmArgs<T>);
  if (p.tile == 64)
    kernel = p.mode == GEMM_RECT ? K_::template get<GEMM_RECT, 64, 4>() : K_::template get<GEMM_LOWER, 64, 4>();
  else if (p.waves == 4)
    kernel = p.mode == GEMM_RECT ? K_::template get<GEMM_RECT, 128, 4>() : K_::template get<GEMM_LOWER, 128, 4>();
  else
    kernel = p.mode == GEMM_RECT    ? K_::template get<GEMM_RECT, 128, 8>()
             : p.mode == GEMM_LOWER ? K_::template get<GEMM_LOWER, 128, 8>()
                                    : K_::template get<GEMM_LAUUM, 128, 8>();
  const dim3 gridd(p.gridx, 1, p.gridz), block(p.waves * 64);
  if (e0)
    hipExtLaunchKernelGGL(kernel, gridd, block, 0, s, e0, e1, 0, g);
  else
    GOGP_KLAUNCH(kernel, gridd, block, 0, s, g);
}

}
```

gogp_amd/csrc/gram.hip:

```cpp
#ifndef GOGP_EV
#include <algorithm>

#include "kern_eval.h"

#define GOGP_EV 0
#define GOGP_EVN(name) name
namespace gogp {
#endif

template <bool CROSS, class T>
__global__ __launch_bounds__(256) void GOGP_EVN(gram_kernel)(const DevParams *__restrict__ Pp,
                                                   const double *__restrict__ Rsrc, long nrows,
                                                   const double *__restrict__ Csrc, long ncols,
                                                   T *__restrict__ Out, long ld, int ntc,
                                                   int strip_w, int toff, long bstride) {
  extern __shared__ double sm[];
  const DevParams &P = *cand(Pp, bstride);
  Out = cand(Out, bstride);
  const int D = P.ndim;
  double *Ri = sm;
  double *CjT = sm + 64 * D;
  unsigned long long *Mr = reinterpret_cast<unsigned long long *>(CjT + 64 * D), *Mc = Mr + 64;
  const int tid = threadIdx.x;
  int ti, tj;
  if (CROSS) {
    ti = blockIdx.x / ntc;
    tj = blockIdx.x - ti * ntc;
  } else if (strip_w > 0) {
    ti = blockIdx.x / strip_w;
    tj = blockIdx.x - ti * strip_w;
    if (ti < tj) return;
  } else {
    const int t = blockIdx.x;
    ti = (int)((sqrt(8.0 * (double)t + 1.0) - 1.0) * 0.5);
    while (ti * (ti + 1) / 2 > t) --ti;
    while ((ti + 1) * (ti + 2) / 2 <= t) ++ti;
    tj = t - ti * (ti + 1) / 2;
    ti += toff;
    tj += toff;
  }
  const long r0 = (long)ti * 64, c0 = (long)tj * 64;
  for (int idx = tid; idx < 64 * D; idx += 256) {
    const int r = idx / D, d = idx - r * D;
    Ri[idx] = (r0 + r < nrows) ? Rsrc[(r0 + r) * D + d] : 0.0;
  }
  for (int idx = tid; idx < 64 * D; idx += 256) {
    const int d = idx >> 6, r = idx & 63;
    CjT[idx] = (c0 + r < ncols) ? Csrc[(c0 + r) * D + d] : 0.0;
  }
  if (GOGP_EV) {
    if (tid < 64) Mr[tid] = event_mask(P, (r0 + tid < nrows) ? Rsrc[(r0 + tid) * D + P.ev_axis] : 0.0);
    else if (tid < 128) Mc[tid - 64] = event_mask(P, (c0 + tid - 64 < ncols) ? Csrc[(c0 + tid - 64) * D + P.ev_axis] : 0.0);
  }
  __syncthreads();
  const int tx = tid & 63, ty = tid >> 6;
  const long gj = c0 + tx;
  const double *cj = CjT + tx;
  if (!CROSS && P.nterms == 1 && P.kind[0] != GOGP_K_PERIODIC) {
    const int rbase = __builtin_amdgcn_readfirstlane(ty) * 16;
    const double *xr = Rsrc + (r0 + rbase) * D;
    double s[16];
#pragma unroll
    for (int rr = 0; rr < 16; ++rr) s[rr] = 0.0;
    for (int d = 0; d < D; ++d) {
      const double il = P.inv_len[0][d];
      const double c = cj[d * 64];
#pragma unroll
      for (int rr = 0; rr < 16; ++rr) {
        const double u = (xr[rr * D + d] - c) * il;
        s[rr] += u * u;
      }
    }
    const int kind = P.kind[0];
    const double c0s = P.c[0];
#pragma unroll 2
    for (int rr = 0; rr < 16; ++rr) {
      const long gi = r0 + rbase + rr;
      double k;
      if (gi < nrows && gj < ncols) {
        double f, dfdr2;
        radial_eval(kind, s[rr], f, dfdr2);
        k = 0.0 + c0s * f;
        if (GOGP_EV) k *= event_discount(P, Mr[rbase + rr], Mc[tx]);
        if (gi == gj) k += P.noise_var;
      } else {
        k = (gi == gj) ? 1.0 : 0.0;
      }
      Out[gi * ld + gj] = (T)k;
    }
    return;
  }
#pragma unroll 2
  for (int rr = 0; rr < 16; ++rr) {
    const int r = ty * 16 + rr;
    const long gi = r0 + r;
    const double *ri = Ri + r * D;
    double k;
    if (gi < nrows && gj < ncols) {
      k = simil_value(
          P, [&](int d) { return ri[d]; }, [&](int d) { return cj[d * 64]; });
      if (GOGP_EV) k *= event_discount(P, Mr[r], Mc[tx]);
      if (!CROSS && gi == gj) k += P.noise_var;
    } else {
      k = (!CROSS && gi == gj) ? 1.0 : 0.0;
    }
    Out[gi * ld + gj] = (T)k;
  }
}

template <class T>
__global__ __launch_bounds__(256) void GOGP_EVN(gram_local_kernel)(const DevParams *__restrict__ Pp,
                                                         const double *__restrict__ X, long n,
                                                         T *__restrict__ Out, long ld, int ntc,
// ... 190 lines not shown
  if (i >= npad) return;
  double s = 0.0;
  for (int q = 0; q < nslab; ++q) s += part[(long)q * npad + i];
  r[i] = (i < n) ? (y ? y[i] - s : s) : 0.0;
}

void launch_residual(hipStream_t s, const DevParams *p, int ndim, const double *X, int64_t n,
                     int64_t npad, const double *v, const double *y, double *part, int nslab, double *r,
                     bool radial1, bool ev) {
  const int ntile = (int)(npad / 64);
  const int tps = (ntile + nslab - 1) / nslab;
  const size_t lds = (size_t)(128 * ndim + 64 + 256) * sizeof(double);
  if (ev && radial1)
    GOGP_KLAUNCH((kmatvec_kernel_ev<true>), dim3((unsigned)ntile, (unsigned)nslab), dim3(256), lds + 64 * 8, s, p, X,
                 (long)n, v, (long)npad, tps, part, 0, ntile);
  else if (ev)
    GOGP_KLAUNCH((kmatvec_kernel_ev<false>), dim3((unsigned)ntile, (unsigned)nslab), dim3(256), lds + 64 * 8, s, p, X,
                 (long)n, v, (long)npad, tps, part, 0, ntile);
  else if (radial1)
    GOGP_KLAUNCH(kmatvec_kernel<true>, dim3((unsigned)ntile, (unsigned)nslab), dim3(256), lds, s, p, X, (long)n,
                       v, (long)npad, tps, part, 0, ntile);
  else
    GOGP_KLAUNCH(kmatvec_kernel<false>, dim3((unsigned)ntile, (unsigned)nslab), dim3(256), lds, s, p, X, (long)n,
                       v, (long)npad, tps, part, 0, ntile);
  GOGP_KLAUNCH(kmatvec_finish_kernel, dim3((unsigned)((npad + 255) / 256)), dim3(256), 0, s, part, nslab,
                     (long)npad, (long)n, y, r);
}

void launch_kmatvec_share(hipStream_t s, const DevParams *p, int ndim, const double *X, int64_t n, int64_t npad,
                          const double *v, int part_idx, int nparts, double *part, int nslab, double *out,
                          bool radial1, bool ev) {
  const int ntile = (int)(npad / 64);
  const int per = (ntile + nparts - 1) / nparts;
  const int t0 = std::min(ntile, part_idx * per), t1 = std::min(ntile, (part_idx + 1) * per);
  const int tps = std::max(1, (t1 - t0 + nslab - 1) / nslab);
  const size_t lds = (size_t)(128 * ndim + 64 + 256) * sizeof(double);
  if (ev && radial1)
    GOGP_KLAUNCH((kmatvec_kernel_ev<true>), dim3((unsigned)ntile, (unsigned)nslab), dim3(256), lds + 64 * 8, s, p, X,
                 (long)n, v, (long)npad, tps, part, t0, t1);
  else if (ev)
    GOGP_KLAUNCH((kmatvec_kernel_ev<false>), dim3((unsigned)ntile, (unsigned)nslab), dim3(256), lds + 64 * 8, s, p, X,
                 (long)n, v, (long)npad, tps, part, t0, t1);
  else if (radial1)
    GOGP_KLAUNCH(kmatvec_kernel<true>, dim3((unsigned)ntile, (unsigned)nslab), dim3(256), lds, s, p, X, (long)n,
                       v, (long)npad, tps, part, t0, t1);
  else
    GOGP_KLAUNCH(kmatvec_kernel<false>, dim3((unsigned)ntile, (unsigned)nslab), dim3(256), lds, s, p, X, (long)n,
                       v, (long)npad, tps, part, t0, t1);
  GOGP_KLAUNCH(kmatvec_finish_kernel, dim3((unsigned)((npad + 255) / 256)), dim3(256), 0, s, part, nslab,
                     (long)npad, (long)n, (const double *)nullptr, out);
}

__global__ void prior_kernel(const DevParams *__restrict__ Pp, const double *__restrict__ Z,
                             long m, double *__restrict__ prior) {
  const long j = (long)blockIdx.x * blockDim.x + threadIdx.x;
  if (j >= m) return;
  const DevParams &P = *Pp;
  const double *z = Z + j * P.ndim;
  prior[j] = simil_value(
      P, [&](int d) { return z[d]; }, [&](int d) { return z[d]; });
}

template <class T>
static void gram_lower_t(hipStream_t s, const DevParams *p, int ndim, const double *X, int64_t n,
                         int64_t npad, T *K, int64_t ld, bool ev) {
  const int nt = (int)(npad / 64);
  const int ntiles = nt * (nt + 1) / 2;
  const size_t lds = (size_t)2 * 64 * ndim * sizeof(double);
  if (ev)
    GOGP_KLAUNCH((gram_kernel_ev<false, T>), dim3(ntiles), dim3(256), lds + 128 * 8, s, p, X, (long)n, X, (long)n, K,
                 (long)ld, nt, 0, 0, 0L);
  else
    GOGP_KLAUNCH((gram_kernel<false, T>), dim3(ntiles), dim3(256), lds, s, p, X, (long)n, X,
                       (long)n, K, (long)ld, nt, 0, 0, 0L);
}
void launch_gram_lower(hipStream_t s, const DevParams *p, int ndim, const double *X, int64_t n,
                       int64_t npad, double *K, int64_t ld, bool ev) {
  gram_lower_t(s, p, ndim, X, n, npad, K, ld, ev);
}

template <class T>
static void gram_lower_split_t(hipStream_t s_first, hipStream_t s_rest, const DevParams *p, int ndim,
                               const double *X, int64_t n, int64_t npad, T *K, int64_t ld,
                               int64_t wcols, bool ev) {
  const int nt = (int)(npad / 64);
  int w = (int)(wcols / 64);
  if (w > nt) w = nt;
  const size_t lds = (size_t)2 * 64 * ndim * sizeof(double);
  const unsigned nz = (unsigned)tl_batch.k;
  const int nr = nt - w;
  if (ev) {
    GOGP_KLAUNCH((gram_kernel_ev<false, T>), dim3(nt * w, 1, nz), dim3(256), lds + 128 * 8, s_first, p, X, (long)n, X,
                 (long)n, K, (long)ld, nt, w, 0, tl_batch.stride);
    if (nr > 0)
      GOGP_KLAUNCH((gram_kernel_ev<false, T>), dim3(nr * (nr + 1) / 2, 1, nz), dim3(256), lds + 128 * 8, s_rest, p, X,
                   (long)n, X, (long)n, K, (long)ld, nt, 0, w, tl_batch.stride);
    return;
  }
  GOGP_KLAUNCH((gram_kernel<false, T>), dim3(nt * w, 1, nz), dim3(256), lds, s_first, p, X, (long)n, X,
                     (long)n, K, (long)ld, nt, w, 0, tl_batch.stride);
  if (nr > 0)
    GOGP_KLAUNCH((gram_kernel<false, T>), dim3(nr * (nr + 1) / 2, 1, nz), dim3(256), lds, s_rest, p, X,
                       (long)n, X, (long)n, K, (long)ld, nt, 0, w, tl_batch.stride);
}
void launch_gram_lower_split(hipStream_t s_first, hipStream_t s_rest, const DevParams *p, int ndim,
                             const double *X, int64_t n, int64_t npad, double *K, int64_t ld,
                             int64_t wcols, bool ev) {
  gram_lower_split_t(s_first, s_rest, p, ndim, X, n, npad, K, ld, wcols, ev);
}
void launch_gram_lower_split(hipStream_t s_first, hipStream_t s_rest, const DevParams *p, int ndim,
                             const double *X, int64_t n, int64_t npad, float *K, int64_t ld,
                             int64_t wcols, bool ev) {
  gram_lower_split_t(s_first, s_rest, p, ndim, X, n, npad, K, ld, wcols, ev);
}

template <class T>
static void gram_local_t(hipStream_t s, const DevParams *p, int ndim, const double *X, int64_t n,
                         int64_t mrows, int64_t ncols, BlockMap map, T *K, int64_t ld, bool ev) {
  const int ntr = (int)(mrows / 64), ntc = (int)(ncols / 64);
  if (ntr <= 0 || ntc <= 0) return;
  const size_t lds = (size_t)2 * 64 * ndim * sizeof(double);
  if (ev)
    GOGP_KLAUNCH((gram_local_kernel_ev<T>), dim3(ntr * ntc), dim3(256), lds + 128 * 8, s, p, X, (long)n, K, (long)ld,
                 ntc, map);
  else
    GOGP_KLAUNCH(gram_local_kernel<T>, dim3(ntr * ntc), dim3(256), lds, s, p, X, (long)n, K, (long)ld,
                       ntc, map);
}
void launch_gram_local(hipStream_t s, const DevParams *p, int ndim, const double *X, int64_t n,
                       int64_t mrows, int64_t ncols, BlockMap map, double *K, int64_t ld, bool ev) {
  gram_local_t(s, p, ndim, X, n, mrows, ncols, map, K, ld, ev);
}
void launch_gram_local(hipStream_t s, const DevParams *p, int ndim, const double *X, int64_t n,
                       int64_t mrows, int64_t ncols, BlockMap map, float *K, int64_t ld, bool ev) {
  gram_local_t(s, p, ndim, X, n, mrows, ncols, map, K, ld, ev);
}

template <class T>
static void cross_t(hipStream_t s, const DevParams *p, int ndim, const double *X, int64_t n,
                    int64_t npad, const double *Z, int64_t m, int64_t mpad, T *KsT, int64_t ld, bool ev) {
  const int ntr = (int)(mpad / 64), ntc = (int)(npad / 64);
  const size_t lds = (size_t)2 * 64 * ndim * sizeof(double);
  if (ev)
    GOGP_KLAUNCH((gram_kernel_ev<true, T>), dim3(ntr * ntc), dim3(256), lds + 128 * 8, s, p, Z, (long)m, X, (long)n, KsT,
                 (long)ld, ntc, 0, 0, 0L);
  else
    GOGP_KLAUNCH((gram_kernel<true, T>), dim3(ntr * ntc), dim3(256), lds, s, p, Z, (long)m, X,
                       (long)n, KsT, (long)ld, ntc, 0, 0, 0L);
}
void launch_cross(hipStream_t s, const DevParams *p, int ndim, const double *X, int64_t n,
                  int64_t npad, const double *Z, int64_t m, int64_t mpad, double *KsT, int64_t ld, bool ev) {
  cross_t(s, p, ndim, X, n, npad, Z, m, mpad, KsT, ld, ev);
}
void launch_cross(hipStream_t s, const DevParams *p, int ndim, const double *X, int64_t n,
                  int64_t npad, const double *Z, int64_t m, int64_t mpad, float *KsT, int64_t ld, bool ev) {
  cross_t(s, p, ndim, X, n, npad, Z, m, mpad, KsT, ld, ev);
}

void launch_prior(hipStream_t s, const DevParams *p, const double *Z, int64_t m,
                  double *prior) {
  if (m <= 0) return;
  GOGP_KLAUNCH(prior_kernel, dim3((unsigned)((m + 255) / 256)), dim3(256), 0, s, p, Z,
                     (long)m, prior);
}

}
#endif
```

gogp_amd/csrc/handle.h:

```cpp
#pragma once
#include <algorithm>
#include <array>
#include <string>
#include <vector>

#include "common.h"

namespace gogp {
struct Dist2D;
}
using gogp::DevParams;
using gogp::GemmProfile;

constexpr int REFINE_SLABS = 8;

constexpr int HS_INFO = 8;
constexpr int HS_TRACE = 9;
constexpr int HS_TMO = 10;
constexpr int HS_PIVOT = 12;
constexpr int HS_GRAD = 16;
static_assert(HS_INFO < HS_TMO && HS_TMO < HS_PIVOT && HS_PIVOT < HS_GRAD, "the staging words lie below the gradient's sums");
static_assert(HS_GRAD + gogp::NACC == gogp::BATCH_ROW, "the pinned row is a batch row");

struct EvalBufs {
// ... 38 lines not shown
struct CandGraphKey {
  int k = 0;
  int64_t n = 0, cap_npad = 0;
  size_t stride = 0;
  const void *arena = nullptr, *dX = nullptr, *dy = nullptr, *hostP = nullptr, *hscal = nullptr;
  bool operator==(const CandGraphKey &o) const {
    return k == o.k && n == o.n && cap_npad == o.cap_npad && stride == o.stride && arena == o.arena && dX == o.dX &&
           dy == o.dy && hostP == o.hostP && hscal == o.hscal;
  }
};

struct gogp_handle : EvalBufs, EvalState {
  gogp_desc desc;
  int device = 0;
  int ns = 0, nn = 0, P = 0, D = 0;
  int ard_dims = 0;
  bool radial1 = false;
  int nevents = 0, ev_axis = 0;
  double events[GOGP_MAX_EVENTS][3] = {};
  bool ev() const { return nevents > 0; }
  int64_t n = 0, npad = 0;
  int nblk = 0;
  double *dX = nullptr, *dy = nullptr;
  double *dscr = nullptr;
  double *D64 = nullptr;
  int64_t cap_d64 = 0;
  int diag_fp64 = 1;
  bool d64_active = false;
  int prec = 64;
  size_t esz() const { return prec == 32 ? sizeof(float) : sizeof(double); }
  int refine_steps = 1;
  double *rw = nullptr, *rz = nullptr, *rd = nullptr, *rpart = nullptr;
  DevParams *hostP = nullptr;
  double *hscal = nullptr;
  int64_t cap_npad = 0;
  int64_t cap_y = 0;
  double *dZ = nullptr, *KsT = nullptr, *Vt = nullptr, *pvec = nullptr;
  int64_t cap_m = 0, cap_mp_npad = 0;
  Workspace pg_ws;
  Workspace pc_ws;
  int ncu = 0;
  hipStream_t s = nullptr;
  hipStream_t sp = nullptr;
  char *cand_arena = nullptr;
  size_t cand_stride = 0;
  int cand_cap_k = 0;
  int64_t cand_cap_npad = 0;
  DevParams *cand_hostP = nullptr;
  double *cand_hscal = nullptr;
  int cand_host_k = 0;
  int batch_k = 1;
  bool batch_mode = false;
  int use_graph = 1;
  bool graph_failed = false;
  int graph_nodes = 0;
  std::string graph_note;
  hipGraphExec_t cand_graph = nullptr;
  hipStream_t sg = nullptr;
  CandGraphKey cand_graph_key, cand_seen_key;
  double *bt_X = nullptr, *bt_y = nullptr;
  int64_t bt_rows = 0, bt_cap_rows = 0;
  std::vector<int64_t> bt_off, bt_n;
  bool bt_have = false;
  char *bt_din = nullptr, *bt_hin = nullptr;
  size_t bt_in_cap = 0;
  double *bt_dout = nullptr, *bt_hout = nullptr;
  size_t bt_out_cap = 0;
  gogp::Dist2D *dist = nullptr;
  hipStream_t sl = nullptr;
  hipStream_t s2 = nullptr;
  hipStream_t st = nullptr;
  hipStream_t sk = nullptr;
  void *stream_set = nullptr;
  std::vector<hipEvent_t> evs;
  int lookahead = 1;
  int superpanel = 2;
  int eager = 1;
  int superpanel_head = -1;
  int head_remaining = 16;
  int chain_prio = -1;
  int tiny = 1;
  int chain_slabs = 0;
  int chain_split = -1;
  int ktri = 1;
  double *TX = nullptr, *Tmt = nullptr;
  int64_t tinv_ld = 0;
  size_t cap_tinv = 0;
  int grad_prec = 64;
  float *g32A = nullptr, *g32L = nullptr, *g32Y = nullptr, *g32D = nullptr;
  int64_t g32_cap = 0;
  int produce_panels = 4;
  int produce_small_below = 1024;
  int produce_tinv = 1;
  bool tinv_valid = false, tinv_pending = false;
  int64_t tinv_sig = 0;
  int produce_small_max = 64;
  Workspace small_ws;
  int produce_groups = 2;
  int krag = 1;
  int ard_mfma_min = 1;
  int kinv_split = 60;
  int64_t kinv_c1 = 0;
  int kinv_fused = -1;
  bool kinv_pending = false;
  bool trtri_pending = false;
  bool ydone_valid = false;
  bool alpha_pending = false;
  std::vector<double> theta_s, theta_n;
  bool have_data = false;
  bool have_theta = false;
  bool z_valid = false;
  Workspace app_ws;
  Workspace rm_ws;
  Workspace loo_vec;
  Workspace loo_mat;
  double yta = 0.0;
  int trace_fp64 = 1;
  double cond_limit = 1e16;
  std::vector<double> grad_cache;
  std::string err;
  GemmProfile prof;
  std::vector<hipEvent_t> aux_ev[GOGP_PROF_NCLASS];
  size_t aux_used[GOGP_PROF_NCLASS] = {0, 0, 0, 0};
};

struct AuxTimer {
  gogp_handle *h;
  int cls;
  hipStream_t s;
  hipEvent_t e1 = nullptr;
  AuxTimer(gogp_handle *h_, int cls_, hipStream_t s_) : h(h_), cls(cls_), s(s_) {
    if (!h->prof.on || cls < 0 || cls >= GOGP_PROF_NCLASS) return;
    auto &pool = h->aux_ev[cls];
    size_t &used = h->aux_used[cls];
    while (pool.size() < used + 2) {
      hipEvent_t e = nullptr;
      (void)hipEventCreate(&e);
      pool.push_back(e);
    }
    (void)hipEventRecord(pool[used], s);
    e1 = pool[used + 1];
    used += 2;
  }
  ~AuxTimer() {
    if (e1) (void)hipEventRecord(e1, s);
  }
};

#define HIPCHK(h, call)                                                                \
  do {                                                                                 \
    hipError_t e_ = (call);                                                            \
    if (e_ != hipSuccess) {                                                            \
      char buf_[512];                                                                  \
      snprintf(buf_, sizeof buf_, "%s failed: %s (%s:%d)", #call, hipGetErrorString(e_), \
               __FILE__, __LINE__);                                                    \
      (h)->err = buf_;                                                                 \
      (void)hipGetLastError();  \
      return (e_ == hipErrorOutOfMemory) ? GOGP_ENOMEM : GOGP_EHIP;                     \
    }                                                                                  \
  } while (0)

inline int Workspace::reserve(gogp_handle *h, size_t need) {
  if (p && bytes >= need) return GOGP_OK;
  release();
  HIPCHK(h, hipMalloc(&p, need));
  bytes = need;
// ... 75 lines not shown
```

gogp_amd/csrc/sgemm.hip:

```cpp
#include "gemm_tile.h"

namespace gogp {

typedef float f32x16 __attribute__((ext_vector_type(16)));
typedef float f32x4 __attribute__((ext_vector_type(4)));

template <int MODE, int BT, int NW>
__global__ __launch_bounds__(NW * 64, NW / 2) void sgemm_nt_kernel(GemmArgs<float> g) {
  constexpr int MT = BT / 64;
  constexpr int NTW = (NW == 8) ? 1 : BT / 64;
  constexpr int WT = BT / 2;
  constexpr int WTN = (NW == 8) ? BT / 4 : BT / 2;
  constexpr int NQ = BT * 8 / (NW * 64);
  constexpr int SROWS = NW * 8;
  __shared__ __attribute__((aligned(16))) float lds[2][2][BT * SGEMM_BK];
  const int tid = threadIdx.x;
  const int lane = tid & 63;
  const int wid = __builtin_amdgcn_readfirstlane(tid >> 6);
  if (g.prio) raise_wave_priority();

  int ti, tj, kbeg, nkt;
  float beta;
  if constexpr (MODE == GEMM_RECT) {
    if (!rect_tile_assignment<BT, SGEMM_BK>(g, ti, tj, beta, kbeg, nkt)) return;
  } else {
    int t = blockIdx.x;
    if (MODE != GEMM_LAUUM) t = xcd_chunk(t);
    ti = (int)((sqrt(8.0 * (double)t + 1.0) - 1.0) * 0.5);
    while (ti * (ti + 1) / 2 > t) --ti;
    while ((ti + 1) * (ti + 2) / 2 <= t) ++ti;
    tj = t - ti * (ti + 1) / 2;
    beta = g.beta;
    if (MODE == GEMM_LOWER && ti >= g.new_row0) beta = 0.0f;
    kbeg = 0, nkt = g.nkt;
    if (MODE != GEMM_LAUUM && ti > g.krag0) {
      kbeg = (ti - g.krag0) * BT;
      nkt -= kbeg / SGEMM_BK;
    }
    if (MODE == GEMM_LAUUM) {
      kbeg = ti * BT;
      nkt = (g.kend - kbeg) / SGEMM_BK;
      if (nkt <= 0) return;
    }
  }
  const float *Ag = g.A + (long)ti * BT * g.lda + kbeg;
  const float *Bg = g.B + (long)tj * BT * g.ldb + kbeg;

  const int srow = tid >> 3;
  const int schunk = tid & 7;
  const int gchunk = schunk ^ ((srow >> 1) & 7);
  const float *Ap = Ag + (long)srow * g.lda + gchunk * 4;
  const float *Bp = Bg + (long)srow * g.ldb + gchunk * 4;
  const long a_step = (long)SROWS * g.lda, b_step = (long)SROWS * g.ldb;

  const int wr = (NW == 8) ? wid >> 2 : wid >> 1;
  const int wc = (NW == 8) ? wid & 3 : wid & 1;
  const int frow = lane & 31, fh = lane >> 5;
  const int abase = (wr * WT + frow) * SGEMM_BK;
  const int bbase = (wc * WTN + frow) * SGEMM_BK;
  int xc[4];
#pragma unroll
  for (int c = 0; c < 4; ++c) xc[c] = ((2 * c + fh) ^ ((frow >> 1) & 7)) << 2;

  float *Cg = g.C + (long)(ti * BT + wr * WT) * g.ldc + tj * BT + wc * WTN;
  const int coff = (4 * fh) * (int)g.ldc + frow;
  const float alpha = g.alpha;

#pragma unroll
  for (int q = 0; q < NQ; ++q) {
    load16_to_lds(Ap + q * a_step, &lds[0][0][(wid * 8 + SROWS * q) * SGEMM_BK]);
    load16_to_lds(Bp + q * b_step, &lds[0][1][(wid * 8 + SROWS * q) * SGEMM_BK]);
  }
  f32x16 acc[MT][NTW];
  if (beta != 0.0f) {
    const float sc = beta / alpha;
#pragma unroll
    for (int m = 0; m < MT; ++m)
#pragma unroll
      for (int n = 0; n < NTW; ++n)
#pragma unroll
        for (int v = 0; v < 16; ++v)
          acc[m][n][v] = sc * (Cg + (long)(m * 32 + (v & 3) + 8 * (v >> 2)) * g.ldc)[coff + n * 32];
  } else {
#pragma unroll
    for (int m = 0; m < MT; ++m)
#pragma unroll
      for (int n = 0; n < NTW; ++n)
#pragma unroll
        for (int v = 0; v < 16; ++v) acc[m][n][v] = 0.0f;
  }
  wait_vmcnt0();
  __syncthreads();

  int cur = 0;
  for (int kt = 0; kt < nkt; ++kt) {
    const bool more = (kt + 1 < nkt);
    if (more) {
      const float *ap = Ap + (long)(kt + 1) * SGEMM_BK;
      const float *bp = Bp + (long)(kt + 1) * SGEMM_BK;
#pragma unroll
      for (int q = 0; q < NQ; ++q) {
        load16_to_lds(ap + q * a_step, &lds[cur ^ 1][0][(wid * 8 + SROWS * q) * SGEMM_BK]);
        load16_to_lds(bp + q * b_step, &lds[cur ^ 1][1][(wid * 8 + SROWS * q) * SGEMM_BK]);
      }
    }
    const float *la = lds[cur][0];
    const float *lb = lds[cur][1];
#pragma unroll
    for (int c = 0; c < 4; ++c) {
      f32x4 a[MT], b[NTW];
#pragma unroll
      for (int m = 0; m < MT; ++m) a[m] = *reinterpret_cast<const f32x4 *>(la + abase + m * 32 * SGEMM_BK + xc[c]);
#pragma unroll
      for (int n = 0; n < NTW; ++n) b[n] = *reinterpret_cast<const f32x4 *>(lb + bbase + n * 32 * SGEMM_BK + xc[c]);
#pragma unroll
      for (int j = 0; j < 4; ++j)
#pragma unroll
        for (int m = 0; m < MT; ++m)
#pragma unroll
          for (int n = 0; n < NTW; ++n)
            acc[m][n] = __builtin_amdgcn_mfma_f32_32x32x2f32(a[m][j], b[n][j], acc[m][n], 0, 0, 0);
    }
    if (more) wait_vmcnt0();
    __syncthreads();
    cur ^= 1;
  }

#pragma unroll
  for (int m = 0; m < MT; ++m)
#pragma unroll
    for (int n = 0; n < NTW; ++n)
#pragma unroll
      for (int v = 0; v < 16; ++v)
        (Cg + (long)(m * 32 + (v & 3) + 8 * (v >> 2)) * g.ldc)[coff + n * 32] = alpha * acc[m][n][v];
}

template <>
struct TileKernel<float> {
  template <int MODE, int BT, int NW>
  static auto get() {
    return &sgemm_nt_kernel<MODE, BT, NW>;
  }
};

void launch_gemm_nt(hipStream_t s, GemmMode mode, int mt, int nt, int64_t K, double alpha, const float *A,
                    int64_t lda, const float *B, int64_t ldb, double beta, float *C, int64_t ldc,
                    GemmProfile *prof, const GemmGrid *grid) {
  launch_tile_gemm<float>(s, mode, mt, nt, K, alpha, A, lda, B, ldb, beta, C, ldc, prof, grid);
}

void launch_gemm_nt(hipStream_t s, GemmMode mode, int mt, int nt, int64_t K, double alpha, const double *A,
                    int64_t lda, const double *B, int64_t ldb, double beta, double *C, int64_t ldc,
                    GemmProfile *prof, const GemmGrid *grid) {
  launch_dgemm_nt(s, mode, mt, nt, K, alpha, A, lda, B, ldb, beta, C, ldc, prof, grid);
}

}
```

gogp_amd/csrc/solve.hip:

```cpp
#include "common.h"

namespace gogp {

__device__ __forceinline__ void load8(const double *p, double *o) {
  const double2 *q = reinterpret_cast<const double2 *>(p);
  const double2 a = q[0], b = q[1], c = q[2], d = q[3];
  o[0] = a.x; o[1] = a.y; o[2] = b.x; o[3] = b.y; o[4] = c.x; o[5] = c.y; o[6] = d.x; o[7] = d.y;
}
__device__ __forceinline__ void load8(const float *p, double *o) {
  const float4 *q = reinterpret_cast<const float4 *>(p);
  const float4 a = q[0], b = q[1];
  o[0] = a.x; o[1] = a.y; o[2] = a.z; o[3] = a.w; o[4] = b.x; o[5] = b.y; o[6] = b.z; o[7] = b.w;
}
__device__ __forceinline__ void load2(const double *p, double &a, double &b) {
  const double2 v = *reinterpret_cast<const double2 *>(p);
  a = v.x;
  b = v.y;
}
__device__ __forceinline__ void load2(const float *p, double &a, double &b) {
  const float2 v = *reinterpret_cast<const float2 *>(p);
  a = v.x;
  b = v.y;
}
__device__ __forceinline__ void store2zero(double *p) {
// ... 281 lines not shown
}

template <class T>
__global__ __launch_bounds__(256) void trace_rows_kernel(const T *__restrict__ Y, long ld, long ncols,
                                                         const double *__restrict__ alpha, double *__restrict__ part) {
  __shared__ double red[4];
  const long i = blockIdx.x;
  const long q0 = (i / PANEL) * PANEL;
  const T *row = Y + i * ld;
  double b = 0.0;
  for (long q = q0 + threadIdx.x; q < ncols; q += 256) {
    const double v = (double)row[q];
    b += v * v;
  }
  b = wave_sum(b);
  if ((threadIdx.x & 63) == 0) red[threadIdx.x >> 6] = b;
  __syncthreads();
  if (threadIdx.x == 0) part[i] = alpha[i] * alpha[i] - ((red[0] + red[1]) + (red[2] + red[3]));
}
__global__ __launch_bounds__(1024) void sum_kernel(const double *__restrict__ v, long n, double *__restrict__ out) {
  __shared__ double red[16];
  double a = 0.0;
  for (long i = threadIdx.x; i < n; i += 1024) a += v[i];
  a = wave_sum(a);
  if ((threadIdx.x & 63) == 0) red[threadIdx.x >> 6] = a;
  __syncthreads();
  if (threadIdx.x == 0) {
    double t = 0.0;
    for (int w = 0; w < 16; ++w) t += red[w];
    out[0] = t;
  }
}
void launch_trace_from_y(hipStream_t s, const float *Y, int64_t ld, int64_t n, int64_t npad, const double *alpha,
                         double *part, double *out) {
  if (n <= 0) return;
  GOGP_KLAUNCH(trace_rows_kernel<float>, dim3((unsigned)n), dim3(256), 0, s, Y, (long)ld, (long)npad, alpha, part);
  GOGP_KLAUNCH(sum_kernel, dim3(1), dim3(1024), 0, s, (const double *)part, (long)n, out);
}

template <class T>
__global__ __launch_bounds__(256) void zero_upper_kernel(T *__restrict__ R, long ld,
                                                         long npad, long bstride) {
  R = cand(R, bstride);
  const long row = blockIdx.y;
  const long cstart = (row / PANEL + 1) * PANEL;
  const long c = cstart + ((long)blockIdx.x * 256 + threadIdx.x) * 2;
  if (c >= npad) return;
  store2zero(R + row * ld + c);
}

void launch_zero_upper_blocks(hipStream_t s, double *R, int64_t ld, int64_t npad) {
  if (npad <= PANEL) return;
  dim3 grid((unsigned)((npad / 2 + 255) / 256), (unsigned)(npad - PANEL), (unsigned)tl_batch.k);
  GOGP_KLAUNCH(zero_upper_kernel<double>, grid, dim3(256), 0, s, R, (long)ld, (long)npad,
                     tl_batch.stride);
}
void launch_zero_upper_blocks(hipStream_t s, float *R, int64_t ld, int64_t npad) {
  if (npad <= PANEL) return;
  dim3 grid((unsigned)((npad / 2 + 255) / 256), (unsigned)(npad - PANEL));
  GOGP_KLAUNCH(zero_upper_kernel<float>, grid, dim3(256), 0, s, R, (long)ld, (long)npad, 0L);
}

template <class T>
__global__ __launch_bounds__(256) void ydiag_kernel(const T *__restrict__ Dinv,
                                                    T *__restrict__ Y, long ld, long bstride) {
  Dinv = cand(Dinv, bstride);
  Y = cand(Y, bstride);
  __shared__ T tile[32][33];
  const int bx = blockIdx.x & 7, by = blockIdx.x >> 3;
  const int tx = threadIdx.x & 31, ty = threadIdx.x >> 5;
#pragma unroll
  for (int r = 0; r < 32; r += 8) tile[ty + r][tx] = Dinv[(by * 32 + ty + r) * 256 + bx * 32 + tx];
  __syncthreads();
#pragma unroll
  for (int r = 0; r < 32; r += 8) Y[(long)(bx * 32 + ty + r) * ld + by * 32 + tx] = tile[tx][ty + r];
}

void launch_ydiag(hipStream_t s, const double *Dinv, double *Ydiag, int64_t ld) {
  GOGP_KLAUNCH(ydiag_kernel<double>, dim3(64, 1, (unsigned)tl_batch.k), dim3(256), 0, s, Dinv, Ydiag,
                     (long)ld, tl_batch.stride);
}
void launch_ydiag(hipStream_t s, const float *Dinv, float *Ydiag, int64_t ld) {
  GOGP_KLAUNCH(ydiag_kernel<float>, dim3(64), dim3(256), 0, s, Dinv, Ydiag, (long)ld, 0L);
}

template <class T>
__global__ __launch_bounds__(256) void tinv_init_kernel(const T *__restrict__ Dinv, T *__restrict__ X,
                                                        T *__restrict__ XT, int nsub, long tld, long bstride) {
  Dinv = cand(Dinv, bstride);
  X = cand(X, bstride);
  if (XT) XT = cand(XT, bstride);
  __shared__ T tile[32][33];
  const int tpr = nsub * 8;
  const int bx = blockIdx.x % tpr, by = blockIdx.x / tpr;
  const int I = by >> 3, J = bx >> 3;
  const int tx = threadIdx.x & 31, ty = threadIdx.x >> 5;
  const long r0 = (long)by * 32, c0 = (long)bx * 32;
  if (I == J) {
    const T *D = Dinv + (long)I * 256 * 256 + (long)(by & 7) * 32 * 256 + (bx & 7) * 32;
#pragma unroll
    for (int r = 0; r < 32; r += 8) {
      const T v = D[(ty + r) * 256 + tx];
      X[(r0 + ty + r) * tld + c0 + tx] = v;
      tile[ty + r][tx] = v;
    }
    if (XT) {
      __syncthreads();
      const long tr0 = (long)I * 256 + (long)(bx & 7) * 32, tc0 = (long)I * 256 + (long)(by & 7) * 32;
#pragma unroll
      for (int r = 0; r < 32; r += 8) XT[(tr0 + ty + r) * tld + tc0 + tx] = tile[tx][ty + r];
    }
  } else if (I < J) {
#pragma unroll
    for (int r = 0; r < 32; r += 8) X[(r0 + ty + r) * tld + c0 + tx] = (T)0;
  } else if (XT) {
#pragma unroll
    for (int r = 0; r < 32; r += 8) XT[(r0 + ty + r) * tld + c0 + tx] = (T)0;
  }
}
void launch_tinv_init(hipStream_t s, const double *Dinv, double *X, double *XT, int nsub, int64_t tld) {
  GOGP_KLAUNCH(tinv_init_kernel<double>, dim3(nsub * 8 * nsub * 8, 1, (unsigned)tl_batch.k), dim3(256), 0, s, Dinv,
                     X, XT, nsub, (long)tld, tl_batch.stride);
}
void launch_tinv_init(hipStream_t s, const float *Dinv, float *X, float *XT, int nsub, int64_t tld) {
  GOGP_KLAUNCH(tinv_init_kernel<float>, dim3(nsub * 8 * nsub * 8), dim3(256), 0, s, Dinv, X, XT, nsub, (long)tld, 0L);
}

constexpr int BLOCKMM_MAX = 6;
template <class T>
struct BlockMM {
  const T *A[BLOCKMM_MAX];
  const T *B[BLOCKMM_MAX];
  T *C[BLOCKMM_MAX];
  long lda[BLOCKMM_MAX], ldb[BLOCKMM_MAX], ldc[BLOCKMM_MAX];
  int K[BLOCKMM_MAX];
  double alpha;
  long bstride;
};
typedef double bmm_f64x4 __attribute__((ext_vector_type(4)));
template <class T>
__global__ __launch_bounds__(256, 2) void blockmm_kernel(BlockMM<T> g) {
  constexpr int KC = 32, AS = KC + 1, BS = 64 + 2;
  __shared__ double As[64 * AS];
  __shared__ double Bs[KC * BS];
  const int b = blockIdx.y;
  const T *A = cand(g.A[b], g.bstride);
  const T *B = cand(g.B[b], g.bstride);
  T *C = cand(g.C[b], g.bstride);
  const long lda = g.lda[b], ldb = g.ldb[b], ldc = g.ldc[b];
  const int K = g.K[b];
  const int tid = threadIdx.x, lane = tid & 63, w = tid >> 6;
  const int tr = blockIdx.x >> 2, tc = blockIdx.x & 3;
  A += (long)tr * 64 * lda;
  B += tc * 64;
  C += (long)tr * 64 * ldc + tc * 64;
  const int ar = tid >> 2, ak = (tid & 3) * 8, bk = tid >> 3, bc = (tid & 7) * 8;
  double ra[8], rb[8];
  auto gload = [&](int k0) {
#pragma unroll
    for (int i = 0; i < 8; ++i) ra[i] = (double)A[(long)ar * lda + k0 + ak + i];
#pragma unroll
    for (int i = 0; i < 8; ++i) rb[i] = (double)B[(long)(k0 + bk) * ldb + bc + i];
  };
  bmm_f64x4 acc[4];
#pragma unroll
  for (int n = 0; n < 4; ++n) acc[n] = (bmm_f64x4){0.0, 0.0, 0.0, 0.0};
// ... 436 lines not shown
```

gogp_amd/csrc/testhooks.hip:

```cpp
#include <cstdlib>
#include <cstring>
#include <stdio.h>

#include "common.h"
#include "gemm_plan.h"
#include "../../include/gogp_testhooks.h"

struct gogp_handle;
namespace gogp {
int dist_init_replay(gogp_handle *h, int rank, int nranks, int prow, int pcol);
}
extern "C" int gogp_test_dist_init_replay(void *h, int rank, int nranks, int prow, int pcol) {
  return gogp::dist_init_replay(static_cast<gogp_handle *>(h), rank, nranks, prow, pcol);
}

namespace gogp_th {
void launch_diag256(hipStream_t s, const double *A, int64_t ld, double *Lout, int64_t ldl,
                    double *Dinv, int64_t row0, int64_t nvalid, long long *info);
void launch_diag256_stamped(hipStream_t s, const double *A, double *Lout, double *Dinv,
                            long long *info, unsigned long long *stamps);
void launch_panel128_stamped(hipStream_t s, const double *A, double *Lout, int64_t rows_below, long long *info,
                             unsigned long long *stamps);
}

// ... 125 lines not shown
  const double flops = (double)blocks * 4.0 * (double)iters * 8.0 * 2.0 * 16 * 16 * 4;
  *tflops = flops / (ms * 1e-3) / 1e12;
  unsigned long long h[2] = {0, 0};
  (void)hipMemcpy(h, clk, 16, hipMemcpyDeviceToHost);
  if (cyc_per_mfma) *cyc_per_mfma = (double)h[0] / ((double)iters * 8.0 * 2.0);
  if (clock_mhz) *clock_mhz = h[1] ? (double)h[0] / (double)h[1] * 100.0 : 0.0;
  (void)hipEventDestroy(e0);
  (void)hipEventDestroy(e1);
  (void)hipFree(sink);
  (void)hipFree(clk);
  return GOGP_OK;
}


}

using namespace gogp;

extern "C" int gogp_mfma_f64_peak(int device, int iters, double *tflops, double *cyc_per_mfma,
                                  double *clock_mhz) {
  if (!tflops || iters <= 0) return GOGP_EARG;
  int ndev = 0;
  if (hipGetDeviceCount(&ndev) != hipSuccess || ndev <= 0) return GOGP_EHIP;
  if (device >= 0 && hipSetDevice(device) != hipSuccess) return GOGP_EHIP;
  return mfma_f64_peak(iters, tflops, cyc_per_mfma, clock_mhz);
}

extern "C" int gogp_mfma_f32_peak(int device, int iters, double *tflops, double *cyc_per_mfma,
                                  double *clock_mhz) {
  if (!tflops || iters <= 0) return GOGP_EARG;
  int ndev = 0;
  if (hipGetDeviceCount(&ndev) != hipSuccess || ndev <= 0) return GOGP_EHIP;
  if (device >= 0 && hipSetDevice(device) != hipSuccess) return GOGP_EHIP;
  return mfma_f32_peak(iters, tflops, cyc_per_mfma, clock_mhz);
}

extern "C" int gogp_test_dgemm_nt(int device, int64_t M, int64_t N, int64_t K, double alpha,
                                  const double *A, const double *B, double beta, double *C) {
  if (!A || !B || !C || M <= 0 || N <= 0 || K <= 0) return GOGP_EARG;
  if (M % TILE || N % TILE || K % GEMM_BK) return GOGP_EARG;
  int ndev = 0;
  if (hipGetDeviceCount(&ndev) != hipSuccess || ndev <= 0) return GOGP_EHIP;
  if (device >= 0 && hipSetDevice(device) != hipSuccess) return GOGP_EHIP;
  double *dA = nullptr, *dB = nullptr, *dC = nullptr;
  hipError_t e = hipMalloc(&dA, (size_t)M * K * sizeof(double));
  if (e == hipSuccess) e = hipMalloc(&dB, (size_t)N * K * sizeof(double));
  if (e == hipSuccess) e = hipMalloc(&dC, (size_t)M * N * sizeof(double));
  if (e == hipSuccess) e = hipMemcpy(dA, A, (size_t)M * K * sizeof(double), hipMemcpyHostToDevice);
  if (e == hipSuccess) e = hipMemcpy(dB, B, (size_t)N * K * sizeof(double), hipMemcpyHostToDevice);
  if (e == hipSuccess) e = hipMemcpy(dC, C, (size_t)M * N * sizeof(double), hipMemcpyHostToDevice);
  if (e == hipSuccess) {
    launch_dgemm_nt(0, GEMM_RECT, (int)(M / TILE), (int)(N / TILE), K, alpha, dA, K, dB, K, beta,
                    dC, N, nullptr);
    e = hipDeviceSynchronize();
  }
  if (e == hipSuccess) e = hipMemcpy(C, dC, (size_t)M * N * sizeof(double), hipMemcpyDeviceToHost);
  (void)hipFree(dA);
  (void)hipFree(dB);
  (void)hipFree(dC);
  return e == hipSuccess ? GOGP_OK : GOGP_EHIP;
}

namespace {
bool covers(int64_t len, int64_t off, int64_t ld, int64_t rows, int64_t cols, int64_t k, int64_t stride) {
  if (len <= 0 || off < 0 || ld < cols || rows <= 0 || cols <= 0 || k <= 0 || stride < 0) return false;
  const int64_t hi = off + (k - 1) * stride + (rows - 1) * ld + cols;
  return hi <= len;
}
bool device_ok(int device) {
  int ndev = 0;
  if (hipGetDeviceCount(&ndev) != hipSuccess || ndev <= 0) return false;
  return device < 0 || hipSetDevice(device) == hipSuccess;
}
bool gemm_launch_args_ok(int precision, int mode, int mt, int nt, int64_t K, const gogp_test_gemm_opts &o) {
  if (precision != 64 && precision != 32) return false;
  if (mode < GEMM_RECT || mode > GEMM_TRAP || mt <= 0 || nt <= 0 || K <= 0) return false;
  const int64_t kstep = precision == 64 ? GEMM_BK : SGEMM_BK, al = 16 / (precision / 8);
  if (K % kstep || K > (1 << 30)) return false;
  if ((mode == GEMM_LOWER || mode == GEMM_LAUUM) && mt != nt) return false;
  if (o.k < 1 || o.k > 64 || o.bstride < 0 || o.bstride % al || (o.k > 1 && o.bstride == 0)) return false;
  if (precision == 32 && (o.k > 1 || o.kbeg0 != 0)) return false;
  if (o.kbeg0 < 0 || o.kbeg0 % kstep || o.kbeg0 > K || (o.kbeg0 && mode != GEMM_LAUUM)) return false;
  if (o.new_row0 < -1 || (o.new_row0 >= 0 && mode != GEMM_LOWER)) return false;
  if (o.ktri && mode != GEMM_RECT) return false;
  if (o.krag0 < -1 || (o.krag0 >= 0 && (o.ktri || (mode != GEMM_RECT && mode != GEMM_LOWER)))) return false;
  if (o.krag0 >= 0 && o.krag0 < mt && K < (int64_t)(mt - o.krag0) * TILE) return false;
  if (o.rule < 0 || o.rule > 2 || (o.rule && mode != GEMM_RECT)) return false;
  if (o.rule && (o.tpb_shift < 0 || o.tpb_shift > 8 || o.rblk0 < 0 || o.cblk0 < 0 || o.Pr < 1 || o.Pc < 1 ||
                 o.pr < 0 || o.pr >= o.Pr || o.pc < 0 || o.pc >= o.Pc))
    return false;
  return true;
}
const gogp_test_gemm_opts GEMM_OPTS_DEFAULT = {0, -1, -1, 0, 384, 0, 0, 0, 0, 0, 0, 1, 0, 1, -1, 1, 0};
GemmGrid gemm_grid_of(const gogp_test_gemm_opts &o) {
  GemmGrid g;
  g.ktri = o.ktri;
  g.krag0 = o.krag0;
  g.new_row0 = o.new_row0;
  g.kbeg0 = o.kbeg0;
  g.small_below = o.small_below;
  g.prio = o.prio;
  g.rule = o.rule;
  g.tpb_shift = o.tpb_shift;
  g.rblk0 = o.rblk0;
  g.cblk0 = o.cblk0;
  g.pr = o.pr;
  g.Pr = o.Pr;
  g.pc = o.pc;
  g.Pc = o.Pc;
  g.beta0 = o.beta0;
  return g;
}
}

extern "C" int gogp_test_gemm_plan(int precision, int mode, int mt, int nt, int64_t K, const gogp_test_gemm_opts *opt,
                                   gogp_test_gemm_plan_out *out) {
  const gogp_test_gemm_opts o = opt ? *opt : GEMM_OPTS_DEFAULT;
  if (!out || !gemm_launch_args_ok(precision, mode, mt, nt, K, o)) return GOGP_EARG;
  const GemmGrid g = gemm_grid_of(o);
  const GemmPlan p = gemm_plan((GemmMode)mode, mt, nt, K, &g, o.k, precision == 64 ? GEMM_F64 : GEMM_F32);
  out->tile = p.tile;
  out->waves = p.waves;
  out->grid_x = p.gridx;
  out->grid_z = p.gridz;
  out->flops = p.flops;
  out->tag = p.tag;
  return GOGP_OK;
}

extern "C" int gogp_test_gemm_nt(int device, int precision, int mode, int mt, int nt, int64_t K, double alpha,
                                 double beta, const void *A, int64_t a_len, int64_t a_off, int64_t lda, const void *B,
                                 int64_t b_len, int64_t b_off, int64_t ldb, void *C, int64_t c_len, int64_t c_off,
                                 int64_t ldc, const gogp_test_gemm_opts *opt) {
  const gogp_test_gemm_opts o = opt ? *opt : GEMM_OPTS_DEFAULT;
  if (!A || !B || !C || !gemm_launch_args_ok(precision, mode, mt, nt, K, o)) return GOGP_EARG;
  const int64_t es = precision / 8, al = 16 / es;
  if (alpha == 0.0 || (precision == 32 && (float)alpha == 0.0f)) return GOGP_EARG;
  if (lda % al || ldb % al || ldc % al || a_off % al || b_off % al || c_off % al) return GOGP_EARG;
  const int64_t M = (int64_t)mt * TILE, N = (int64_t)nt * TILE;
  if (!covers(a_len, a_off, lda, M, K, o.k, o.bstride) || !covers(b_len, b_off, ldb, N, K, o.k, o.bstride) ||
      !covers(c_len, c_off, ldc, M, N, o.k, o.bstride))
    return GOGP_EARG;
  if (!device_ok(device)) return GOGP_EHIP;

  char *dA = nullptr, *dB = nullptr, *dC = nullptr;
  hipError_t e = hipMalloc(&dA, (size_t)(a_len * es));
  if (e == hipSuccess) e = hipMalloc(&dB, (size_t)(b_len * es));
  if (e == hipSuccess) e = hipMalloc(&dC, (size_t)(c_len * es));
  if (e == hipSuccess) e = hipMemcpy(dA, A, (size_t)(a_len * es), hipMemcpyHostToDevice);
  if (e == hipSuccess) e = hipMemcpy(dB, B, (size_t)(b_len * es), hipMemcpyHostToDevice);
  if (e == hipSuccess) e = hipMemcpy(dC, C, (size_t)(c_len * es), hipMemcpyHostToDevice);
  if (e == hipSuccess) {
    const GemmGrid g = gemm_grid_of(o);
    tl_batch.k = o.k;
    tl_batch.stride = (long)(o.bstride * es);
    if (precision == 64)
      launch_gemm_nt(0, (GemmMode)mode, mt, nt, K, alpha, (const double *)dA + a_off, lda, (const double *)dB + b_off, ldb,
                     beta, (double *)dC + c_off, ldc, nullptr, &g);
    else
      launch_gemm_nt(0, (GemmMode)mode, mt, nt, K, alpha, (const float *)dA + a_off, lda, (const float *)dB + b_off, ldb,
                     beta, (float *)dC + c_off, ldc, nullptr, &g);
    tl_batch.k = 1;
    tl_batch.stride = 0;
    e = hipGetLastError();
    if (e == hipSuccess) e = hipDeviceSynchronize();
  }
  if (e == hipSuccess) e = hipMemcpy(C, dC, (size_t)(c_len * es), hipMemcpyDeviceToHost);
  (void)hipFree(dA);
  (void)hipFree(dB);
  (void)hipFree(dC);
  return e == hipSuccess ? GOGP_OK : GOGP_EHIP;
}

extern "C" int gogp_test_diag_syrk(int device, int bs, const float *L, int64_t l_len, int64_t l_off, int64_t ld,
                                   int64_t K, int64_t row_stride, double *D64, int64_t d_len, int nblocks) {
  if (!L || !D64 || (bs != PANEL && bs != 2 * PANEL) || nblocks < 1 || nblocks > 4096) return GOGP_EARG;
  if (K < 16 || K % 16 || ld % 4 || l_off % 4 || row_stride % 4) return GOGP_EARG;
  if (bs == PANEL && row_stride != PANEL * ld) return GOGP_EARG;
  if (!covers(l_len, l_off, ld, bs, K, nblocks, row_stride) || d_len < (int64_t)nblocks * bs * bs) return GOGP_EARG;
  if (!device_ok(device)) return GOGP_EHIP;
  float *dL = nullptr;
  double *dD = nullptr;
  hipError_t e = hipMalloc(&dL, (size_t)l_len * sizeof(float));
  if (e == hipSuccess) e = hipMalloc(&dD, (size_t)d_len * sizeof(double));
  if (e == hipSuccess) e = hipMemcpy(dL, L, (size_t)l_len * sizeof(float), hipMemcpyHostToDevice);
  if (e == hipSuccess) e = hipMemcpy(dD, D64, (size_t)d_len * sizeof(double), hipMemcpyHostToDevice);
  if (e == hipSuccess) {
    if (bs == PANEL)
      launch_diag_syrk_f64(0, dL + l_off, ld, K, dD, nblocks);
    else
      launch_diag_syrk_f64_tiles(0, dL + l_off, ld, K, dD, nblocks, row_stride, bs);
    e = hipGetLastError();
    if (e == hipSuccess) e = hipDeviceSynchronize();
  }
  if (e == hipSuccess) e = hipMemcpy(D64, dD, (size_t)d_len * sizeof(double), hipMemcpyDeviceToHost);
  (void)hipFree(dL);
  (void)hipFree(dD);
  return e == hipSuccess ? GOGP_OK : GOGP_EHIP;
}

extern "C" int gogp_test_diag256_product(int device, int variant, const double *A, int64_t ld, double *L, int64_t ldl,
                                         double *Dinv, int64_t row0, int64_t nvalid, long long *info) {
  if (!A || !L || !Dinv || !info || variant < 0 || variant > 3) return GOGP_EARG;
  if (ld < PANEL || ldl < PANEL || ld % 2 || ldl % 2 || row0 < 0 || nvalid < 0) return GOGP_EARG;
  const int64_t ldd = (variant & 1) ? 2 * PANEL : PANEL;
  if (!device_ok(device)) return GOGP_EHIP;
  double *dA = nullptr, *dL = nullptr, *dD = nullptr;
  long long *dinfo = nullptr;
  const size_t na = (size_t)PANEL * ld * 8, nl = (size_t)PANEL * ldl * 8, nd = (size_t)PANEL * ldd * 8;
// ... 714 lines not shown
```

include/gogp_testhooks.h:

```cpp
#ifndef GOGP_TESTHOOKS_H
#define GOGP_TESTHOOKS_H

#include <stdint.h>

#include "gogp_hip.h"

#ifdef __cplusplus
extern "C" {
#endif

int gogp_mfma_f64_peak(int device, int iters, double *tflops, double *cyc_per_mfma,
                       double *clock_mhz);
int gogp_mfma_f32_peak(int device, int iters, double *tflops, double *cyc_per_mfma,
                       double *clock_mhz);

int gogp_test_dgemm_nt(int device, int64_t M, int64_t N, int64_t K, double alpha,
                       const double *A, const double *B, double beta, double *C);

typedef struct gogp_test_gemm_opts {
  int32_t ktri, krag0, new_row0, kbeg0, small_below, prio;
  int32_t rule, tpb_shift, rblk0, cblk0, pr, Pr, pc, Pc, beta0;
  int32_t k;
  int64_t bstride;
} gogp_test_gemm_opts;

int gogp_test_gemm_nt(int device, int precision, int mode, int mt, int nt, int64_t K, double alpha, double beta,
                      const void *A, int64_t a_len, int64_t a_off, int64_t lda, const void *B, int64_t b_len,
                      int64_t b_off, int64_t ldb, void *C, int64_t c_len, int64_t c_off, int64_t ldc,
                      const gogp_test_gemm_opts *opt);

typedef struct gogp_test_gemm_plan_out {
  int32_t tile, waves;
  int64_t grid_x, grid_z;
  double flops;
  int64_t tag;
} gogp_test_gemm_plan_out;
int gogp_test_gemm_plan(int precision, int mode, int mt, int nt, int64_t K, const gogp_test_gemm_opts *opt,
                        gogp_test_gemm_plan_out *out);

int gogp_test_diag_syrk(int device, int bs, const float *L, int64_t l_len, int64_t l_off, int64_t ld, int64_t K,
                        int64_t row_stride, double *D64, int64_t d_len, int nblocks);

int gogp_test_diag256_product(int device, int variant, const double *A, int64_t ld, double *L, int64_t ldl,
                              double *Dinv, int64_t row0, int64_t nvalid, long long *info);


int64_t gogp_test_trsm_small_workspace(int64_t npad);

int gogp_test_trsm_small(int device, int precision, int64_t npad, const void *L, int64_t l_len, int64_t ld,
                         const void *Dinv, const void *KsT, int64_t k_len, int64_t ldk, int j0, int cnt, double *dq,
                         int64_t dq_len, void *sol, int64_t sol_len, int *kind, int *width, int64_t *sol_off,
                         unsigned *tmo);

int gogp_test_trsv_steps(int device, int precision, int dir, int64_t npad, const void *L, int64_t l_len, int64_t ld,
                         const void *Dinv, int b0, int b1, int k, int64_t bstride, double *w, int64_t w_len, double *out,
                         int64_t out_len);

int gogp_test_alpha_from_y(int device, int precision, int64_t npad, const void *Y, int64_t y_len, int64_t ld,
                           const double *z, int64_t z_len, double *alpha, int64_t alpha_len);

int gogp_test_rownorm_dot(int device, int precision, const void *V, int64_t v_len, int64_t ld, int64_t ncols, int64_t m,
                          const double *vec, int64_t vec_len, double *dot, int64_t dot_len, double *sq, int64_t sq_len);

int gogp_test_tinv(int device, int precision, int nsub, const void *Dinv, void *X, int64_t x_len, int64_t tld, int with_xt,
                   void *XT);

int gogp_test_blockmm(int device, int precision, int nprod, void *arena, int64_t arena_len, const int64_t *a_off,
                      const int64_t *lda, const int64_t *b_off, const int64_t *ldb, const int64_t *c_off,
                      const int64_t *ldc, const int *K, double alpha, int k, int64_t bstride);


typedef struct gogp_test_kparams {
  int32_t ndim, nterms;
  int32_t kind[GOGP_MAX_TERMS], ard[GOGP_MAX_TERMS];
  double c[GOGP_MAX_TERMS], w[GOGP_MAX_TERMS], inv_len[GOGP_MAX_TERMS][GOGP_MAX_NDIM];
  double noise_var, dnoise;
  int32_t nevents, ev_axis;
  double ev_from[GOGP_MAX_EVENTS], ev_to[GOGP_MAX_EVENTS], ev_disc[GOGP_MAX_EVENTS];
} gogp_test_kparams;

#define GOGP_TEST_NACC (16 + GOGP_MAX_NDIM)

int gogp_test_grad_blocks(int64_t npad, int64_t mrows, int64_t ncols, int max_blocks);

int gogp_test_grad_reduce(int device, int precision, const gogp_test_kparams *kparams, int ard_dims, int radial1,
                          int mfma_min, int ev, const double *X, int64_t x_len, const double *alpha, int64_t alpha_len,
                          const void *Kinv, int64_t kinv_len, int64_t ld, int64_t n, int64_t npad, int max_blocks, int k,
                          int64_t bstride, double *partials, int64_t partials_len, double *out);

int gogp_test_grad_reduce_local(int device, int precision, const gogp_test_kparams *kparams, int ard_dims, int radial1,
                                int mfma_min, int ev, const double *X, int64_t x_len, const double *alpha,
                                int64_t alpha_len, const void *Kinv, int64_t kinv_len, int64_t ld, int64_t n, int64_t npad,
                                int64_t mrows, int64_t ncols, int nb_shift, int pr, int Pr, int pc, int Pc, int max_blocks,
                                int k, int64_t bstride, double *partials, int64_t partials_len, double *out);

int gogp_test_xgrad(int device, const gogp_test_kparams *kparams, int ev, const double *X, int64_t x_len,
                    const double *alpha, int64_t alpha_len, double *Kinv, int64_t kinv_len, int64_t ld, int64_t n,
                    int64_t npad, double *gx, int64_t gx_len);

int gogp_bench_gemm(int device, int mode, int mt, int nt, int64_t K, int reps,
                    double *ms_per_launch, double *tflops);

int gogp_test_diag256(int device, const double *A, double *Lout, double *Dinv,
                      unsigned long long *stamps, double *elapsed_us);

int gogp_test_valu_cost(int device, double *out8);

int gogp_test_panel128(int device, const double *A, double *Lout, int64_t rows_below, int reps,
                       unsigned long long *stamps, double *elapsed_us);

int gogp_test_panel128_slabs(int device, const double *A, double *Lout, int64_t rows_below, int slabs, int reps,
                             double *elapsed_us);

int gogp_test_dist_init_replay(void *h, int rank, int nranks, int prow, int pcol);

#ifdef __cplusplus
}
#endif
// ... 2 lines not shown
```

Baseline: 13.73.

## Overlap first diagonal block with Gram build and fuse inverse head initialization

Adds a head_tail mode, enabled by default (-1). The first 256x256 Gram block is computed separately so its diagonal factorization can start before the rest of the Gram matrix is built. Per superpanel, the Y diagonal and zero blocks are now written by a single inverse_heads kernel instead of a full zero-fill plus ydiag and zero_block launches. The GEMM gains a first_row0 flag that skips reading C for rows not yet initialized. This removes a full-matrix memset and several small launches, at the cost of extra event synchronization and more complex correctness conditions.

```diff
diff --git a/gogp_amd/_lib.py b/gogp_amd/_lib.py
--- a/gogp_amd/_lib.py
+++ b/gogp_amd/_lib.py
@@ -32,10 +32,11 @@
                                 ctypes.c_int64)
 class CGemmOpts(ctypes.Structure):
     _fields_ = [(n, ctypes.c_int32) for n in ("ktri", "krag0", "new_row0", "kbeg0", "small_below", "prio", "rule",
-                                              "tpb_shift", "rblk0", "cblk0", "pr", "Pr", "pc", "Pc", "beta0", "k")]
+                                              "tpb_shift", "rblk0", "cblk0", "pr", "Pr", "pc", "Pc", "beta0", "k",
+                                              "first_row0")]
     _fields_ += [("bstride", ctypes.c_int64)]
     DEFAULTS = dict(ktri=0, krag0=-1, new_row0=-1, kbeg0=0, small_below=384, prio=0, rule=0, tpb_shift=0, rblk0=0,
-                    cblk0=0, pr=0, Pr=1, pc=0, Pc=1, beta0=-1, k=1, bstride=0)
+                    cblk0=0, pr=0, Pr=1, pc=0, Pc=1, beta0=-1, k=1, first_row0=-1, bstride=0)
 
 
 class CKParams(ctypes.Structure):
@@ -52,7 +53,8 @@
 
 class CGemmPlan(ctypes.Structure):
     _fields_ = [("tile", ctypes.c_int32), ("waves", ctypes.c_int32), ("grid_x", ctypes.c_int64),
-                ("grid_z", ctypes.c_int64), ("flops", ctypes.c_double), ("tag", ctypes.c_int64)]
+                ("grid_z", ctypes.c_int64), ("flops", ctypes.c_double), ("tag", ctypes.c_int64),
+                ("first_row0", ctypes.c_int64)]
 
 
 SYMBOLS = [
diff --git a/gogp_amd/csrc/api.hip b/gogp_amd/csrc/api.hip
--- a/gogp_amd/csrc/api.hip
+++ b/gogp_amd/csrc/api.hip
@@ -643,6 +643,8 @@
   }
 }
 
+static inline bool head_tail_of(const gogp_handle *h) { return h->head_tail != 0; }
+
 template <class T>
 struct InvBufs {
   T *A, *Y;
@@ -656,13 +658,16 @@
   GemmProfile *pf = &h->prof;
   const int P0 = P.P0;
   const int64_t C0 = P.C0(), CE = P.CE();
+  const bool ht = head_tail_of(h);
   for (int q = 0; q < P.nsub; ++q) {
     const int p = P0 + q;
     const int64_t c0 = (int64_t)p * PANEL, c2 = c0 + PANEL;
     const T *Dp = B.Dinv + (size_t)p * PANEL * PANEL;
-    launch_ydiag(st, Dp, Y + c0 * ld + c0, ld);
-    if (c2 < CE)
-      launch_zero_block(st, Y + c2 * ld + c0, ld, CE - c2, PANEL);
+    if (!ht) {
+      launch_ydiag(st, Dp, Y + c0 * ld + c0, ld);
+      if (c2 < CE)
+        launch_zero_block(st, Y + c2 * ld + c0, ld, CE - c2, PANEL);
+    }
     if (c0 > 0) {
       GemmGrid gtri = chain_grid(h);
       gtri.ktri = h->ktri;
@@ -673,6 +678,7 @@
       const InnerGroup g = inner_group(q, c2, CE);
       GemmGrid gch = chain_grid(h);
       if (h->krag) gch.krag0 = (int)(g.k0 / TILE);
+      if (ht) gch.first_row0 = (int)(g.k0 / TILE);
       launch_gemm_nt(st, GEMM_RECT, (int)(c2 / TILE), (int)((g.ce - c2) / TILE), (int64_t)g.grp * PANEL,
                       -1.0, Y + g.k0, ld, L + c2 * ld + g.k0, ld, 1.0, R + c2, ld, pf, &gch);
     }
@@ -687,6 +693,7 @@
       (void)gogp::rec_stream_wait(st, ev(h, EV_BASE + 4 * P.prevP0 + 3));
     GemmGrid gch = chain_grid(h), gbulk;
     if (h->krag) gch.krag0 = gbulk.krag0 = (int)(C0 / TILE);
+    if (ht) gch.first_row0 = gbulk.first_row0 = (int)(C0 / TILE);
     launch_gemm_nt(st, GEMM_RECT, mr, ntn, Kw, -1.0, Y + C0, ld, L + CE * ld + C0, ld, 1.0,
                     R + CE, ld, pf, &gch);
     if (nt > ntn) {
@@ -745,6 +752,15 @@
     launch_zero_upper_blocks(s, reinterpret_cast<T *>(h->bufA), h->npad, h->npad);
 }
 template <class T>
+static void inverse_heads(gogp_handle *h, bool mixed, const SuperPanel &P, hipStream_t q) {
+  const int64_t ld = h->npad, y0 = P.C0() * (ld + 1);
+  const size_t d0 = (size_t)P.P0 * PANEL * PANEL;
+  if (mixed)
+    launch_inverse_heads(q, h->Dinv + d0, h->g32Y + y0, ld, P.nsub);
+  else
+    launch_inverse_heads(q, reinterpret_cast<const T *>(h->Dinv) + d0, reinterpret_cast<T *>(h->bufY) + y0, ld, P.nsub);
+}
+template <class T>
 static void inverse_superstep(gogp_handle *h, bool mixed, const SuperPanel &P, hipStream_t st, hipStream_t s2,
                               bool fuse_kinv) {
   if (mixed) {
@@ -822,6 +838,7 @@
   bool mixed = !fp32 && mixed_gradient(h);
   bool fuse_kinv = eager && (h->kinv_fused < 0 ? (npad <= 10240 || mixed) : h->kinv_fused != 0);
   int split = fp32 ? 0 : chain_split_of(h, eager);
+  bool early_diag = head_tail_of(h) && !split;
 
   void d64_init(hipStream_t q, int first, int nblk) const {
     if constexpr (fp32)
@@ -837,24 +854,35 @@
   int build_gram() const {
     if (sp != s) order(h, EV_ENTRY, s, sp);
     HIPCHK(h, cand_memset(h, h->info, sizeof(long long), sp));
+    if (fp32) HIPCHK(h, hipMemsetAsync(h->scalars + 5, 0, sizeof(double), sp));
     const int w0 = superpanel_width(h, npanel, 0);
-    {
-      AuxTimer tm(h, GOGP_PROF_GRAM, s);
-      launch_gram_lower_split(sp, s, h->devP, h->D, h->dX, h->n, npad, A, ld, (int64_t)w0 * PANEL, h->ev());
-    }
     h->d64_active = fp32 && h->diag_fp64 != 0;
     if (h->d64_active) {
       const int rc = ensure_d64(h);
       if (rc != GOGP_OK) return rc;
-      d64_init(sp, 0, w0);
+    }
+    if (early_diag) {
+      launch_gram_first_block(sp, h->devP, h->D, h->dX, h->n, npad, A, ld, h->ev());
+      if (h->d64_active) d64_init(sp, 0, 1);
+      diag_block(h, sp, A, ld, L, ld, Dinv, 0);
+    }
+    {
+      AuxTimer tm(h, GOGP_PROF_GRAM, s);
+      launch_gram_lower_split(sp, s, h->devP, h->D, h->dX, h->n, npad, A, ld, (int64_t)w0 * PANEL, h->ev(), early_diag);
+    }
+    if (h->d64_active) {
+      if (!early_diag) d64_init(sp, 0, w0);
+      else if (w0 > 1) d64_init(sp, 1, w0 - 1);
       if (npanel > w0) d64_init(s, w0, npanel - w0);
     }
     (void)gogp::rec_event_record(ev(h, EV_GRAM), s);
     if (eager) {
       (void)gogp::rec_stream_wait(s2, ev(h, EV_GRAM));
       (void)gogp::rec_stream_wait(st, ev(h, EV_GRAM));
-      zero_inverse_rhs<T>(h, mixed, s2);
-      order(h, EV_INIT, s2, st);
+      if (!head_tail_of(h)) {
+        zero_inverse_rhs<T>(h, mixed, s2);
+        order(h, EV_INIT, s2, st);
+      }
     }
     return GOGP_OK;
   }
@@ -869,7 +897,7 @@
       }
       if (!split) {
         T *Dp = Dinv + (size_t)p * PANEL * PANEL;
-        diag_block(h, sp, A + c0 * ld + c0, ld, L + c0 * ld + c0, ld, Dp, c0);
+        if (p > 0 || !early_diag) diag_block(h, sp, A + c0 * ld + c0, ld, L + c0 * ld + c0, ld, Dp, c0);
         const int mt2 = (int)((npad - c2) / TILE);
         if (mt2 > 0) {
           GemmGrid gtri = chain_grid(h);
@@ -895,11 +923,13 @@
     if constexpr (!fp32) {
       if (split) {
         launch_dinv256_blocks(sz, L + (int64_t)P.P0 * PANEL * (ld + 1), ld, Dinv + (size_t)P.P0 * PANEL * PANEL, P.nsub);
-        if (eager) {
-          (void)gogp::rec_event_record(ev(h, EV_BASE + 5 * (size_t)npanel + 32 + (size_t)P.P0), sz);
-          (void)gogp::rec_stream_wait(st, ev(h, EV_BASE + 5 * (size_t)npanel + 32 + (size_t)P.P0));
-        }
       }
+    }
+    const bool heads = eager && head_tail_of(h);
+    if (heads) inverse_heads<T>(h, mixed, P, sz);
+    if (eager && (split || heads)) {
+      (void)gogp::rec_event_record(ev(h, EV_BASE + 5 * (size_t)npanel + 32 + (size_t)P.P0), sz);
+      (void)gogp::rec_stream_wait(st, ev(h, EV_BASE + 5 * (size_t)npanel + 32 + (size_t)P.P0));
     }
     for (int q = 0; q < P.nsub; ++q) launch_trsv_fwd_step(sz, L, ld, Dinv, P.P0 + q, npanel, h->w, h->z);
   }
@@ -977,7 +1007,6 @@
   if (rc == GOGP_OK && (c.mixed || c.eager)) rc = c.mixed ? ensure_g32(h) : ensure_y(h);
   if (rc == GOGP_OK) rc = c.build_gram();
   if (rc != GOGP_OK) return rc;
-  if (c.fp32) HIPCHK(h, hipMemsetAsync(h->scalars + 5, 0, sizeof(double), c.sp));
   HIPCHK(h, cand_copy_in(h, h->w, h->dy, (size_t)c.npad * sizeof(double), c.sp));
   if (c.sz != c.sp) order(h, EV_W, c.sp, c.sz);
   for (const SuperPanel &P : superpanels(h)) {
@@ -1151,9 +1180,12 @@
     hipStream_t sp = h->lookahead ? h->sp : h->s;
     const int rcy = mixed ? ensure_g32(h) : ensure_y(h);
     if (rcy != GOGP_OK) return rcy;
-    zero_inverse_rhs<T>(h, mixed, s);
+    if (!head_tail_of(h)) zero_inverse_rhs<T>(h, mixed, s);
     order(h, EV_INIT, s, sp);
-    for (const SuperPanel &P : superpanels(h)) inverse_superstep<T>(h, mixed, P, sp, s, false);
+    for (const SuperPanel &P : superpanels(h)) {
+      if (head_tail_of(h)) inverse_heads<T>(h, mixed, P, sp);
+      inverse_superstep<T>(h, mixed, P, sp, s, false);
+    }
     order(h, EV_TRTRI, sp, s);
     h->trtri_done = true;
   } else if (h->trtri_pending) {
@@ -2918,6 +2950,11 @@
     h->ktri = value != 0;
     return GOGP_OK;
   }
+  if (strcmp(name, "head_tail") == 0) {
+    if (value < -1 || value > 0) return fail(h, GOGP_EARG, "head_tail must be -1 or 0");
+    h->head_tail = (int)value;
+    return GOGP_OK;
+  }
   if (strcmp(name, "graph") == 0) {
     if (value < 0 || value > 3) return fail(h, GOGP_EARG, "graph must be 0..3");
     h->use_graph = (int)value;
diff --git a/gogp_amd/csrc/common.h b/gogp_amd/csrc/common.h
--- a/gogp_amd/csrc/common.h
+++ b/gogp_amd/csrc/common.h
@@ -54,6 +54,7 @@
 struct GemmGrid {
   int rule = 0, tpb_shift = 0, rblk0 = 0, cblk0 = 0, pr = 0, Pr = 1, pc = 0, Pc = 1, beta0 = -1;
   int new_row0 = -1;
+  int first_row0 = -1;
   int ktri = 0;
   int prio = 0;
   int krag0 = -1;
@@ -100,7 +101,9 @@
                     GemmProfile *prof, const GemmGrid *grid = nullptr);
 void launch_gram_lower_split(hipStream_t s_first, hipStream_t s_rest, const DevParams *p, int ndim,
                              const double *X, int64_t n, int64_t npad, float *K, int64_t ld,
-                             int64_t wcols, bool ev = false);
+                             int64_t wcols, bool ev = false, bool skip_first = false);
+void launch_gram_first_block(hipStream_t s, const DevParams *p, int ndim, const double *X, int64_t n, int64_t npad,
+                             float *K, int64_t ld, bool ev = false);
 void launch_cross(hipStream_t s, const DevParams *p, int ndim, const double *X, int64_t n,
                   int64_t npad, const double *Z, int64_t m, int64_t mpad, float *KsT, int64_t ld, bool ev = false);
 void launch_trsv_fwd_step(hipStream_t s, const float *L, int64_t ld, const float *Dinv, int b, int nblk,
@@ -135,7 +138,9 @@
                        int64_t mrows, int64_t ncols, BlockMap map, float *K, int64_t ld, bool ev = false);
 void launch_gram_lower_split(hipStream_t s_first, hipStream_t s_rest, const DevParams *p, int ndim,
                              const double *X, int64_t n, int64_t npad, double *K, int64_t ld,
-                             int64_t wcols, bool ev = false);
+                             int64_t wcols, bool ev = false, bool skip_first = false);
+void launch_gram_first_block(hipStream_t s, const DevParams *p, int ndim, const double *X, int64_t n, int64_t npad,
+                             double *K, int64_t ld, bool ev = false);
 void launch_cross(hipStream_t s, const DevParams *p, int ndim, const double *X, int64_t n,
                   int64_t npad, const double *Z, int64_t m, int64_t mpad, double *KsT,
                   int64_t ld, bool ev = false);
@@ -236,6 +241,9 @@
                          int64_t npad, double *alpha);
 void launch_zero_block(hipStream_t s, double *B, int64_t ld, int64_t rows, int64_t cols);
 void launch_ydiag(hipStream_t s, const double *Dinv, double *Ydiag, int64_t ld);
+void launch_inverse_heads(hipStream_t s, const double *Dinv, double *Y, int64_t ld, int nsub);
+void launch_inverse_heads(hipStream_t s, const float *Dinv, float *Y, int64_t ld, int nsub);
+void launch_inverse_heads(hipStream_t s, const double *Dinv, float *Y, int64_t ld, int nsub);
 void launch_tinv_init(hipStream_t s, const double *Dinv, double *X, double *XT, int nsub, int64_t tld);
 void launch_tinv_init(hipStream_t s, const float *Dinv, float *X, float *XT, int nsub, int64_t tld);
 void launch_blockmm(hipStream_t s, int nprod, const double *const *A, const int64_t *lda, const double *const *B,
diff --git a/gogp_amd/csrc/dgemm.hip b/gogp_amd/csrc/dgemm.hip
--- a/gogp_amd/csrc/dgemm.hip
+++ b/gogp_amd/csrc/dgemm.hip
@@ -153,7 +153,8 @@
     load16_to_lds(Bp + q * b_step, &lds[0][1][(wid * 8 + SROWS * q) * GEMM_BK]);
   }
   f64x4 acc[MT][NTW];
-  if (beta != 0.0) {
+  const bool first = MODE == GEMM_RECT && ti >= g.first_row0;
+  if (beta != 0.0 && !first) {
     const double sc = beta / alpha;
 #pragma unroll
     for (int m = 0; m < MT; ++m)
@@ -163,10 +164,11 @@
         for (int v = 0; v < 4; ++v)
           acc[m][n][v] = sc * (Cg + (long)(m * 16 + 4 * v) * g.ldc)[coff + n * 16];
   } else {
+    const double z = beta != 0.0 ? (beta / alpha) * 0.0 : 0.0;
 #pragma unroll
     for (int m = 0; m < MT; ++m)
 #pragma unroll
-      for (int n = 0; n < NTW; ++n) acc[m][n] = (f64x4){0.0, 0.0, 0.0, 0.0};
+      for (int n = 0; n < NTW; ++n) acc[m][n] = (f64x4){z, z, z, z};
   }
   wait_vmcnt0();
   __syncthreads();
diff --git a/gogp_amd/csrc/gemm_plan.h b/gogp_amd/csrc/gemm_plan.h
--- a/gogp_amd/csrc/gemm_plan.h
+++ b/gogp_amd/csrc/gemm_plan.h
@@ -16,6 +16,7 @@
 
 struct GemmPlan {
   int mt, nt, nkt, kend, trap, rule, tpb_shift, rblk0, cblk0, pr, Pr, pc, Pc, beta0, new_row0, ktri, prio, krag0;
+  int first_row0;
   int kbeg0;
   GemmMode mode;
   int ntiles;
@@ -37,6 +38,7 @@
   p.rule = p.tpb_shift = p.rblk0 = p.cblk0 = p.pr = p.pc = p.beta0 = 0;
   p.Pr = p.Pc = 1;
   p.new_row0 = (mode == GEMM_LOWER && grid && grid->new_row0 >= 0) ? grid->new_row0 : NONE;
+  p.first_row0 = (mode == GEMM_RECT && grid && !grid->rule && grid->first_row0 >= 0) ? grid->first_row0 : NONE;
   p.ktri = (mode == GEMM_RECT && grid && grid->ktri) ? 1 : 0;
   p.prio = grid ? grid->prio : 0;
   p.krag0 = (mode != GEMM_LAUUM && mode != GEMM_TRAP && grid && grid->krag0 >= 0 && !p.ktri) ? grid->krag0 : NONE;
@@ -113,6 +115,7 @@
     p.nt = nt * 2;
     p.tpb_shift += 1;
     if (p.new_row0 != NONE) p.new_row0 *= 2;
+    if (p.first_row0 != NONE) p.first_row0 *= 2;
     if (p.krag0 != NONE) p.krag0 *= 2;
     p.gridx = (mode == GEMM_RECT) ? (p.rule ? 8 * ((p.mt + 7) / 8) * p.nt : p.mt * p.nt) : p.mt * (p.mt + 1) / 2;
   }
diff --git a/gogp_amd/csrc/gemm_tile.h b/gogp_amd/csrc/gemm_tile.h
--- a/gogp_amd/csrc/gemm_tile.h
+++ b/gogp_amd/csrc/gemm_tile.h
@@ -24,6 +24,7 @@
   int ktri;
   int prio;
   int krag0;
+  int first_row0;
 };
 template <class T>
 struct GemmArgs : GemmArgsCommon<T> {};
@@ -116,7 +117,7 @@
   g.mt = p.mt, g.nt = p.nt, g.nkt = p.nkt, g.kend = p.kend, g.trap = p.trap;
   g.rule = p.rule, g.tpb_shift = p.tpb_shift, g.rblk0 = p.rblk0, g.cblk0 = p.cblk0, g.beta0 = p.beta0;
   g.pr = p.pr, g.Pr = p.Pr, g.pc = p.pc, g.Pc = p.Pc;
-  g.new_row0 = p.new_row0, g.ktri = p.ktri, g.prio = p.prio, g.krag0 = p.krag0;
+  g.new_row0 = p.new_row0, g.ktri = p.ktri, g.prio = p.prio, g.krag0 = p.krag0, g.first_row0 = p.first_row0;
   if constexpr (F64) {
     g.kbeg0 = p.kbeg0;
     g.bstride = tl_batch.stride;
diff --git a/gogp_amd/csrc/gram.hip b/gogp_amd/csrc/gram.hip
--- a/gogp_amd/csrc/gram.hip
+++ b/gogp_amd/csrc/gram.hip
@@ -29,6 +29,7 @@
   } else if (strip_w > 0) {
     ti = blockIdx.x / strip_w;
     tj = blockIdx.x - ti * strip_w;
+    ti += toff;
     if (ti < tj) return;
   } else {
     const int t = blockIdx.x;
@@ -385,36 +386,61 @@
 template <class T>
 static void gram_lower_split_t(hipStream_t s_first, hipStream_t s_rest, const DevParams *p, int ndim,
                                const double *X, int64_t n, int64_t npad, T *K, int64_t ld,
-                               int64_t wcols, bool ev) {
+                               int64_t wcols, bool ev, bool skip_first) {
   const int nt = (int)(npad / 64);
   int w = (int)(wcols / 64);
   if (w > nt) w = nt;
   const size_t lds = (size_t)2 * 64 * ndim * sizeof(double);
   const unsigned nz = (unsigned)tl_batch.k;
   const int nr = nt - w;
+  const int r0 = skip_first ? (int)(PANEL / 64) : 0;
   if (ev) {
-    GOGP_KLAUNCH((gram_kernel_ev<false, T>), dim3(nt * w, 1, nz), dim3(256), lds + 128 * 8, s_first, p, X, (long)n, X,
-                 (long)n, K, (long)ld, nt, w, 0, tl_batch.stride);
+    if (nt > r0)
+      GOGP_KLAUNCH((gram_kernel_ev<false, T>), dim3((nt - r0) * w, 1, nz), dim3(256), lds + 128 * 8, s_first, p, X, (long)n,
+                   X, (long)n, K, (long)ld, nt, w, r0, tl_batch.stride);
     if (nr > 0)
       GOGP_KLAUNCH((gram_kernel_ev<false, T>), dim3(nr * (nr + 1) / 2, 1, nz), dim3(256), lds + 128 * 8, s_rest, p, X,
                    (long)n, X, (long)n, K, (long)ld, nt, 0, w, tl_batch.stride);
     return;
   }
-  GOGP_KLAUNCH((gram_kernel<false, T>), dim3(nt * w, 1, nz), dim3(256), lds, s_first, p, X, (long)n, X,
-                     (long)n, K, (long)ld, nt, w, 0, tl_batch.stride);
+  if (nt > r0)
+    GOGP_KLAUNCH((gram_kernel<false, T>), dim3((nt - r0) * w, 1, nz), dim3(256), lds, s_first, p, X, (long)n, X,
+                 (long)n, K, (long)ld, nt, w, r0, tl_batch.stride);
   if (nr > 0)
     GOGP_KLAUNCH((gram_kernel<false, T>), dim3(nr * (nr + 1) / 2, 1, nz), dim3(256), lds, s_rest, p, X,
                        (long)n, X, (long)n, K, (long)ld, nt, 0, w, tl_batch.stride);
 }
 void launch_gram_lower_split(hipStream_t s_first, hipStream_t s_rest, const DevParams *p, int ndim,
                              const double *X, int64_t n, int64_t npad, double *K, int64_t ld,
-                             int64_t wcols, bool ev) {
-  gram_lower_split_t(s_first, s_rest, p, ndim, X, n, npad, K, ld, wcols, ev);
+                             int64_t wcols, bool ev, bool skip_first) {
+  gram_lower_split_t(s_first, s_rest, p, ndim, X, n, npad, K, ld, wcols, ev, skip_first);
 }
 void launch_gram_lower_split(hipStream_t s_first, hipStream_t s_rest, const DevParams *p, int ndim,
                              const double *X, int64_t n, int64_t npad, float *K, int64_t ld,
-                             int64_t wcols, bool ev) {
-  gram_lower_split_t(s_first, s_rest, p, ndim, X, n, npad, K, ld, wcols, ev);
+                             int64_t wcols, bool ev, bool skip_first) {
+  gram_lower_split_t(s_first, s_rest, p, ndim, X, n, npad, K, ld, wcols, ev, skip_first);
+}
+
+template <class T>
+static void gram_first_block_t(hipStream_t s, const DevParams *p, int ndim, const double *X, int64_t n, int64_t npad, T *K,
+                               int64_t ld, bool ev) {
+  const int nt = (int)(npad / 64), w = (int)(PANEL / 64);
+  const size_t lds = (size_t)2 * 64 * ndim * sizeof(double);
+  const unsigned nz = (unsigned)tl_batch.k;
+  if (ev)
+    GOGP_KLAUNCH((gram_kernel_ev<false, T>), dim3(w * w, 1, nz), dim3(256), lds + 128 * 8, s, p, X, (long)n, X, (long)n, K,
+                 (long)ld, nt, w, 0, tl_batch.stride);
+  else
+    GOGP_KLAUNCH((gram_kernel<false, T>), dim3(w * w, 1, nz), dim3(256), lds, s, p, X, (long)n, X, (long)n, K, (long)ld, nt,
+                 w, 0, tl_batch.stride);
+}
+void launch_gram_first_block(hipStream_t s, const DevParams *p, int ndim, const double *X, int64_t n, int64_t npad,
+                             double *K, int64_t ld, bool ev) {
+  gram_first_block_t(s, p, ndim, X, n, npad, K, ld, ev);
+}
+void launch_gram_first_block(hipStream_t s, const DevParams *p, int ndim, const double *X, int64_t n, int64_t npad,
+                             float *K, int64_t ld, bool ev) {
+  gram_first_block_t(s, p, ndim, X, n, npad, K, ld, ev);
 }
 
 template <class T>
diff --git a/gogp_amd/csrc/handle.h b/gogp_amd/csrc/handle.h
--- a/gogp_amd/csrc/handle.h
+++ b/gogp_amd/csrc/handle.h
@@ -144,6 +144,7 @@
   int tiny = 1;
   int chain_slabs = 0;
   int chain_split = -1;
+  int head_tail = -1;
   int ktri = 1;
   double *TX = nullptr, *Tmt = nullptr;
   int64_t tinv_ld = 0;
diff --git a/gogp_amd/csrc/sgemm.hip b/gogp_amd/csrc/sgemm.hip
--- a/gogp_amd/csrc/sgemm.hip
+++ b/gogp_amd/csrc/sgemm.hip
@@ -72,7 +72,8 @@
     load16_to_lds(Bp + q * b_step, &lds[0][1][(wid * 8 + SROWS * q) * SGEMM_BK]);
   }
   f32x16 acc[MT][NTW];
-  if (beta != 0.0f) {
+  const bool first = MODE == GEMM_RECT && ti >= g.first_row0;
+  if (beta != 0.0f && !first) {
     const float sc = beta / alpha;
 #pragma unroll
     for (int m = 0; m < MT; ++m)
@@ -82,12 +83,13 @@
         for (int v = 0; v < 16; ++v)
           acc[m][n][v] = sc * (Cg + (long)(m * 32 + (v & 3) + 8 * (v >> 2)) * g.ldc)[coff + n * 32];
   } else {
+    const float z = beta != 0.0f ? (beta / alpha) * 0.0f : 0.0f;
 #pragma unroll
     for (int m = 0; m < MT; ++m)
 #pragma unroll
       for (int n = 0; n < NTW; ++n)
 #pragma unroll
-        for (int v = 0; v < 16; ++v) acc[m][n][v] = 0.0f;
+        for (int v = 0; v < 16; ++v) acc[m][n][v] = z;
   }
   wait_vmcnt0();
   __syncthreads();
diff --git a/gogp_amd/csrc/solve.hip b/gogp_amd/csrc/solve.hip
--- a/gogp_amd/csrc/solve.hip
+++ b/gogp_amd/csrc/solve.hip
@@ -387,6 +387,41 @@
 }
 void launch_ydiag(hipStream_t s, const float *Dinv, float *Ydiag, int64_t ld) {
   GOGP_KLAUNCH(ydiag_kernel<float>, dim3(64), dim3(256), 0, s, Dinv, Ydiag, (long)ld, 0L);
+}
+
+template <class TD, class TY>
+__global__ __launch_bounds__(256) void inverse_heads_kernel(const TD *__restrict__ Dinv, TY *__restrict__ Y, long ld,
+                                                            int nsub, long bstride) {
+  const int br = blockIdx.y / nsub, bc = blockIdx.y - br * nsub;
+  if (br < bc) return;
+  Dinv = cand(Dinv, bstride) + (long)bc * PANEL * PANEL;
+  Y = cand(Y, bstride) + (long)br * PANEL * ld + (long)bc * PANEL;
+  const int bx = blockIdx.x & 7, by = blockIdx.x >> 3;
+  const int tx = threadIdx.x & 31, ty = threadIdx.x >> 5;
+  if (br > bc) {
+#pragma unroll
+    for (int r = 0; r < 32; r += 8) Y[(long)(bx * 32 + ty + r) * ld + by * 32 + tx] = TY(0);
+    return;
+  }
+  __shared__ TY tile[32][33];
+#pragma unroll
+  for (int r = 0; r < 32; r += 8) tile[ty + r][tx] = (TY)Dinv[(by * 32 + ty + r) * 256 + bx * 32 + tx];
+  __syncthreads();
+#pragma unroll
+  for (int r = 0; r < 32; r += 8) Y[(long)(bx * 32 + ty + r) * ld + by * 32 + tx] = tile[tx][ty + r];
+}
+
+void launch_inverse_heads(hipStream_t s, const double *Dinv, double *Y, int64_t ld, int nsub) {
+  GOGP_KLAUNCH((inverse_heads_kernel<double, double>), dim3(64, (unsigned)(nsub * nsub), (unsigned)tl_batch.k), dim3(256), 0,
+               s, Dinv, Y, (long)ld, nsub, tl_batch.stride);
+}
+void launch_inverse_heads(hipStream_t s, const float *Dinv, float *Y, int64_t ld, int nsub) {
+  GOGP_KLAUNCH((inverse_heads_kernel<float, float>), dim3(64, (unsigned)(nsub * nsub)), dim3(256), 0, s, Dinv, Y, (long)ld,
+               nsub, 0L);
+}
+void launch_inverse_heads(hipStream_t s, const double *Dinv, float *Y, int64_t ld, int nsub) {
+  GOGP_KLAUNCH((inverse_heads_kernel<double, float>), dim3(64, (unsigned)(nsub * nsub)), dim3(256), 0, s, Dinv, Y, (long)ld,
+               nsub, 0L);
 }
 
 template <class T>
diff --git a/gogp_amd/csrc/testhooks.hip b/gogp_amd/csrc/testhooks.hip
--- a/gogp_amd/csrc/testhooks.hip
+++ b/gogp_amd/csrc/testhooks.hip
@@ -231,6 +231,7 @@
   if (precision == 32 && (o.k > 1 || o.kbeg0 != 0)) return false;
   if (o.kbeg0 < 0 || o.kbeg0 % kstep || o.kbeg0 > K || (o.kbeg0 && mode != GEMM_LAUUM)) return false;
   if (o.new_row0 < -1 || (o.new_row0 >= 0 && mode != GEMM_LOWER)) return false;
+  if (o.first_row0 < -1 || (o.first_row0 >= 0 && (mode != GEMM_RECT || o.rule))) return false;
   if (o.ktri && mode != GEMM_RECT) return false;
   if (o.krag0 < -1 || (o.krag0 >= 0 && (o.ktri || (mode != GEMM_RECT && mode != GEMM_LOWER)))) return false;
   if (o.krag0 >= 0 && o.krag0 < mt && K < (int64_t)(mt - o.krag0) * TILE) return false;
@@ -240,12 +241,13 @@
     return false;
   return true;
 }
-const gogp_test_gemm_opts GEMM_OPTS_DEFAULT = {0, -1, -1, 0, 384, 0, 0, 0, 0, 0, 0, 1, 0, 1, -1, 1, 0};
+const gogp_test_gemm_opts GEMM_OPTS_DEFAULT = {0, -1, -1, 0, 384, 0, 0, 0, 0, 0, 0, 1, 0, 1, -1, 1, -1, 0};
 GemmGrid gemm_grid_of(const gogp_test_gemm_opts &o) {
   GemmGrid g;
   g.ktri = o.ktri;
   g.krag0 = o.krag0;
   g.new_row0 = o.new_row0;
+  g.first_row0 = o.first_row0;
   g.kbeg0 = o.kbeg0;
   g.small_below = o.small_below;
   g.prio = o.prio;
@@ -274,6 +276,7 @@
   out->grid_z = p.gridz;
   out->flops = p.flops;
   out->tag = p.tag;
+  out->first_row0 = p.first_row0 == 0x7fffffff ? -1 : p.first_row0;
   return GOGP_OK;
 }
 
diff --git a/include/gogp_testhooks.h b/include/gogp_testhooks.h
--- a/include/gogp_testhooks.h
+++ b/include/gogp_testhooks.h
@@ -21,6 +21,7 @@
   int32_t ktri, krag0, new_row0, kbeg0, small_below, prio;
   int32_t rule, tpb_shift, rblk0, cblk0, pr, Pr, pc, Pc, beta0;
   int32_t k;
+  int32_t first_row0;
   int64_t bstride;
 } gogp_test_gemm_opts;
 
@@ -34,6 +35,7 @@
   int64_t grid_x, grid_z;
   double flops;
   int64_t tag;
+  int64_t first_row0;
 } gogp_test_gemm_plan_out;
 int gogp_test_gemm_plan(int precision, int mode, int mt, int nt, int64_t K, const gogp_test_gemm_opts *opt,
                         gogp_test_gemm_plan_out *out);
```

After: 13.85 (median of 6 runs). About the same (+0.8%).
